# Chemical118/TREW

Measured on AMD Instinct MI355X. Metric: Gbases/s scanned (short 5 32, 150 bp reads), higher is better.
Workload: dtype u32

## Files before the change

### include/trew_hip.h

```cpp
#ifndef TREW_HIP_H
#define TREW_HIP_H

#include <stddef.h>
#include <stdint.h>

#ifdef __cplusplus
extern "C" {
#endif

#define TREW_HIP_ABI_VERSION 4

enum {
    TREW_MODE_SHORT = 0,
    TREW_MODE_PAIR = 1,
    TREW_MODE_LONG = 2,
    TREW_MODE_SEGMENT = 3
};

enum {
    TREW_TABLE_FORWARD_HIGH = 0,
    TREW_TABLE_FORWARD_LOW = 1,
    TREW_TABLE_BACKWARD_HIGH = 2,
    TREW_TABLE_BACKWARD_LOW = 3,
    TREW_TABLE_BOTH_HIGH = 4,
    TREW_TABLE_BOTH_LOW = 5,
    TREW_NUM_TABLES = 6
};

enum {
    TREW_FLAG_NO_FILTER = 1,
    TREW_FLAG_DEBUG_NO_EMIT = 2,
    TREW_FLAG_DEBUG_NO_KLOOP = 4,
    TREW_FLAG_DEBUG_POISON_LDS = 32,
    TREW_FLAG_DEBUG_WIDE_NO_WAIT = 128,
    TREW_FLAG_NO_TIMING = 64,
    TREW_FLAG_COMPAT_G1 = 512,
    TREW_FLAG_DEBUG_NO_JOINT = 2048,
    TREW_FLAG_DEBUG_NO_UNI_DRAIN = 4096,
    TREW_FLAG_DEBUG_NO_GROUP = 1024,
    TREW_FLAG_DEBUG_ANNOT_GENERAL = 8192,
    TREW_FLAG_DEBUG_SMALL_BOUNDS = 16384,
    TREW_FLAG_TRACK_PRESSURE = 256
};

typedef struct {
    int32_t min_mer;
    int32_t max_mer;
    double low_baseline;
    double high_baseline;
    int32_t slice_length;
    int32_t mode;
    int32_t device;
    int32_t n_slots;
    uint64_t max_batch_words;
    uint64_t max_batch_reads;
    uint32_t table_log2_slots;
    uint32_t flags;
    uint64_t max_batch_ascii_bytes;
} trew_hip_params;

typedef struct {
    const uint32_t *words;
    uint64_t n_words;
    const uint32_t *offsets;
    const uint32_t *lengths;
    uint32_t uniform_length;
    uint32_t uniform_stride;
    uint64_t n_reads;
    int32_t on_device;
    int32_t max_length;
} trew_hip_batch;

typedef struct {
    const char *bases;
    uint64_t n_bytes;
    const uint32_t *byte_offsets;
    const uint32_t *lengths;
    const uint32_t *word_offsets;
    uint32_t uniform_length;
    uint32_t reserved;
    uint64_t n_reads;
} trew_hip_ascii_batch;

typedef struct {
    int32_t k;
    int32_t table;
    uint64_t word_lo;
    uint64_t word_hi;
    uint64_t count;
} trew_hip_row;

typedef struct trew_hip_ctx trew_hip_ctx;

int trew_hip_init(const trew_hip_params *params, trew_hip_ctx **out);
void trew_hip_destroy(trew_hip_ctx *ctx);
const char *trew_hip_last_error(const trew_hip_ctx *ctx);

int trew_hip_submit(trew_hip_ctx *ctx, const trew_hip_batch *batch, int slot);
int trew_hip_submit_ascii(trew_hip_ctx *ctx, const trew_hip_ascii_batch *batch, int slot);
int trew_hip_pack_ascii(trew_hip_ctx *ctx, const trew_hip_ascii_batch *batch, uint32_t *words, uint64_t words_cap, uint64_t *n_words);
int trew_hip_wait(trew_hip_ctx *ctx, int slot);

int trew_hip_collect(trew_hip_ctx *ctx, int table, trew_hip_row *rows, uint64_t cap, uint64_t *n_rows);
int trew_hip_reset_tables(trew_hip_ctx *ctx);
int trew_hip_add_rows(trew_hip_ctx *ctx, const trew_hip_row *rows, uint64_t n_rows);

int trew_hip_collect_device(trew_hip_ctx *ctx, trew_hip_row *d_rows, uint64_t cap, uint64_t *n_rows);
int trew_hip_add_rows_device(trew_hip_ctx *ctx, const trew_hip_row *d_rows, uint64_t n_rows);
int trew_hip_merge(trew_hip_ctx *dst, trew_hip_ctx *src);
int trew_hip_add_gathered_device(trew_hip_ctx *ctx, const trew_hip_row *d_buf, uint32_t n_slices, uint32_t own_slice,
                                 uint64_t slice_rows, void *producer_stream, uint64_t *max_rows);
int trew_hip_collect_slice_device(trew_hip_ctx *ctx, trew_hip_row *d_slice, uint64_t slice_rows, void *consumer_stream, uint64_t *n_rows);

int trew_hip_table_pressure(trew_hip_ctx *ctx, uint64_t *used_slots, uint64_t *total_slots, uint64_t *spilled_rows,
                            uint64_t *spill_capacity);

#define TREW_DEBUG_COUNTERS 10
int trew_hip_debug_counters(trew_hip_ctx *ctx, uint64_t *out, int n);

int trew_hip_debug_worklist(trew_hip_ctx *ctx, int slot, uint32_t *units, uint64_t cap, uint64_t *n);

int trew_hip_segment_results(trew_hip_ctx *ctx, int slot, int32_t *k_high, int32_t *k_low,
                             uint64_t *seq_high, uint64_t *seq_low, uint64_t *seq_high_hi, uint64_t *seq_low_hi,
                             uint64_t n_reads);
int trew_hip_filter_masks(trew_hip_ctx *ctx, const trew_hip_batch *batch, uint64_t *cand, int slots_per_read);

int trew_hip_last_timing(trew_hip_ctx *ctx, int slot, float *ms_filter, float *ms_exact, uint64_t *n_flagged);

typedef struct {
    int32_t k;
    int32_t reserved;
    uint64_t word;
} trew_hip_motif;
typedef struct {
    uint32_t windows_fwd, windows_rev, tract_start_fwd, tract_len_fwd, tract_start_rev, tract_len_rev;
} trew_hip_annot;
#define TREW_ANNOT_MAX_MOTIFS 8

int trew_motif_parse(const char *text, trew_hip_motif *out);
int trew_hip_annotate(trew_hip_ctx *ctx, const trew_hip_batch *batch, int slot, const trew_hip_motif *motifs, int n_motifs);
int trew_hip_annotate_results(trew_hip_ctx *ctx, int slot, trew_hip_annot *out, uint64_t cap, uint64_t *n, float *ms_kernel);
int trew_annotate_host(const uint32_t *words, const uint32_t *offsets, const uint32_t *lengths, uint64_t n_reads,
                       const trew_hip_motif *motifs, int n_motifs, trew_hip_annot *out);

typedef struct {
    uint32_t covered_fwd, head_len_fwd, head_cov_fwd, tail_len_fwd, tail_cov_fwd;
    uint32_t covered_rev, head_len_rev, head_cov_rev, tail_len_rev, tail_cov_rev;
} trew_hip_tract;
int trew_hip_tracts(trew_hip_ctx *ctx, const trew_hip_batch *batch, int slot, const trew_hip_motif *motifs, int n_motifs, int penalty);
int trew_hip_tracts_results(trew_hip_ctx *ctx, int slot, trew_hip_tract *out, uint64_t cap, uint64_t *n, float *ms_kernel);
int trew_tracts_host(const uint32_t *words, const uint32_t *offsets, const uint32_t *lengths, uint64_t n_reads,
                     const trew_hip_motif *motifs, int n_motifs, int penalty, trew_hip_tract *out);

typedef struct {
    uint32_t max_gap, min_len;
} trew_hip_interval_rule;
typedef struct {
    uint32_t read, motif, strand, start, end, covered;
} trew_hip_interval;
int trew_hip_intervals(trew_hip_ctx *ctx, const trew_hip_batch *batch, int slot, const trew_hip_motif *motifs, const trew_hip_interval_rule *rules,
                       int n_motifs, uint64_t max_intervals);
int trew_hip_intervals_results(trew_hip_ctx *ctx, int slot, trew_hip_interval *out, uint64_t cap, uint64_t *n, uint32_t *counts, float *ms_kernel);
int trew_intervals_host(const uint32_t *words, const uint32_t *offsets, const uint32_t *lengths, uint64_t n_reads, const trew_hip_motif *motifs,
                        const trew_hip_interval_rule *rules, int n_motifs, trew_hip_interval *out, uint64_t cap, uint64_t *n, uint32_t *counts);

#define TREW_VARIANT_BINS 128
#define TREW_VARIANT_NONE 0xffffffffu
typedef struct {
    uint32_t units_fwd, variants_fwd, distinct_fwd, top_fwd, top_count_fwd;
    uint32_t units_rev, variants_rev, distinct_rev, top_rev, top_count_rev;
} trew_hip_variant;
int trew_hip_variants(trew_hip_ctx *ctx, const trew_hip_batch *batch, int slot, const trew_hip_motif *motifs, int n_motifs);
int trew_hip_variants_results(trew_hip_ctx *ctx, int slot, trew_hip_variant *out, uint64_t cap, uint64_t *n, uint64_t *hist, uint64_t *reads_with,
                              float *ms_kernel);
int trew_variants_host(const uint32_t *words, const uint32_t *offsets, const uint32_t *lengths, uint64_t n_reads, const trew_hip_motif *motifs,
                       int n_motifs, trew_hip_variant *out, uint64_t *hist, uint64_t *reads_with);

typedef struct {
    uint32_t period, scored_period, score, start, end, matches, support, reserved;
    uint64_t unit;
} trew_hip_period;
int trew_hip_periods(trew_hip_ctx *ctx, const trew_hip_batch *batch, int slot, int min_period, int max_period, int penalty, uint32_t min_score);
int trew_hip_periods_results(trew_hip_ctx *ctx, int slot, trew_hip_period *out, uint64_t cap, uint64_t *n, float *ms_kernel);
int trew_periods_host(const uint32_t *words, const uint32_t *offsets, const uint32_t *lengths, uint64_t n_reads, int min_period, int max_period,
                      int penalty, uint32_t min_score, trew_hip_period *out);

typedef struct {
    uint32_t read, motif, strand, start, count, bin;
} trew_hip_chain_item;
int trew_hip_chain(trew_hip_ctx *ctx, const trew_hip_batch *batch, int slot, const trew_hip_motif *motifs, int n_motifs, uint64_t max_events);
int trew_hip_chain_results(trew_hip_ctx *ctx, int slot, trew_hip_chain_item *out, uint64_t cap, uint64_t *n_items, uint64_t *n_events,
                           uint32_t *counts, float *ms_kernel);
int trew_chain_host(const uint32_t *words, const uint32_t *offsets, const uint32_t *lengths, uint64_t n_reads, const trew_hip_motif *motifs,
                    int n_motifs, trew_hip_chain_item *out, uint64_t cap, uint64_t *n_items, uint32_t *counts);

typedef struct {
    uint32_t read, depth, period, scored_period, score, start, end, matches, support, reserved;
    uint64_t unit;
} trew_hip_repeat;
int trew_hip_repeats(trew_hip_ctx *ctx, const trew_hip_batch *batch, int slot, int min_period, int max_period, int penalty, uint32_t min_score,
                     uint64_t max_records);
int trew_hip_repeats_results(trew_hip_ctx *ctx, int slot, trew_hip_repeat *out, uint64_t cap, uint64_t *n, uint32_t *counts, float *ms_kernel);
int trew_repeats_host(const uint32_t *words, const uint32_t *offsets, const uint32_t *lengths, uint64_t n_reads, int min_period, int max_period,
// ... 99 lines not shown
```

### trew_amd/__init__.py

```python
from . import capi
from .capi import (
    FLAG_NO_FILTER,
    FLAG_DEBUG_ANNOT_GENERAL,
    FLAG_DEBUG_POISON_LDS,
    FLAG_NO_TIMING,
    FLAG_TRACK_PRESSURE,
    FLAG_COMPAT_G1,
    FLAG_DEBUG_NO_GROUP,
    FLAG_DEBUG_NO_JOINT,
    FLAG_DEBUG_NO_UNI_DRAIN,
    FLAG_DEBUG_SMALL_BOUNDS,
    FLAG_DEBUG_WIDE_NO_WAIT,
    MODE_LONG,
    MODE_PAIR,
    MODE_SEGMENT,
    MODE_SHORT,
    TABLE_NAMES,
    TrewHip,
    TrewHipError,
    align,
    annotate,
    chain,
    decompose,
    intervals,
    k_mer_check,
    pack_reads,
    periods,
    refine,
    repeats,
    satellites,
    tandems,
    trace,
    tracts,
    variants,
)
```

### trew_amd/capi.py

```python
from __future__ import annotations

import ctypes as C
import os

import numpy as np

_HERE = os.path.dirname(os.path.abspath(__file__))
LIB_PATH = os.environ.get("TREW_HIP_LIB") or os.path.join(_HERE, "lib", "libtrew_hip.so")

MODE_SHORT, MODE_PAIR, MODE_LONG, MODE_SEGMENT = 0, 1, 2, 3
FLAG_NO_FILTER = 1
FLAG_DEBUG_POISON_LDS = 32
FLAG_NO_TIMING = 64
FLAG_COMPAT_G1 = 512
FLAG_TRACK_PRESSURE = 256
FLAG_DEBUG_NO_JOINT = 2048
FLAG_DEBUG_NO_UNI_DRAIN = 4096
FLAG_DEBUG_NO_GROUP = 1024
FLAG_DEBUG_ANNOT_GENERAL = 8192
FLAG_DEBUG_SMALL_BOUNDS = 16384
FLAG_DEBUG_WIDE_NO_WAIT = 128
TABLE_NAMES = ("forward_high", "forward_low", "backward_high", "backward_low", "both_high", "both_low")

EXPORTED_SYMBOLS = (
    "trew_hip_init", "trew_hip_destroy", "trew_hip_last_error", "trew_hip_submit", "trew_hip_wait",
    "trew_hip_collect", "trew_hip_reset_tables", "trew_hip_add_rows", "trew_hip_segment_results",
    "trew_hip_filter_masks", "trew_hip_last_timing", "trew_pack_words", "trew_pack_reads",
    "trew_synth_short_ascii", "trew_synth_short_device", "trew_synth_pair_ascii", "trew_synth_pair_device",
    "trew_hip_malloc", "trew_hip_free", "trew_hip_memcpy_h2d", "trew_hip_memcpy_d2h", "trew_hip_abi_version",
    "trew_pack_pairs", "trew_hip_host_alloc", "trew_hip_host_free", "trew_hip_device_count",
    "trew_synth_long_lengths", "trew_synth_long_ascii", "trew_synth_long_device",
    "trew_hip_collect_device", "trew_hip_add_rows_device", "trew_hip_merge", "trew_hip_table_pressure",
    "trew_hip_add_gathered_device", "trew_hip_collect_slice_device", "trew_hip_debug_counters", "trew_hip_debug_worklist", "trew_hip_submit_ascii", "trew_hip_pack_ascii",
    "trew_motif_parse", "trew_hip_annotate", "trew_hip_annotate_results", "trew_annotate_host",
    "trew_hip_tracts", "trew_hip_tracts_results", "trew_tracts_host",
    "trew_hip_intervals", "trew_hip_intervals_results", "trew_intervals_host",
    "trew_hip_variants", "trew_hip_variants_results", "trew_variants_host",
    "trew_hip_periods", "trew_hip_periods_results", "trew_periods_host",
    "trew_hip_chain", "trew_hip_chain_results", "trew_chain_host",
    "trew_hip_repeats", "trew_hip_repeats_results", "trew_repeats_host",
    "trew_hip_satellites", "trew_hip_satellites_results", "trew_satellites_host",
    "trew_hip_align", "trew_hip_align_results", "trew_align_host",
    "trew_hip_refine", "trew_hip_refine_results", "trew_refine_host",
    "trew_hip_tandems", "trew_hip_tandems_results", "trew_tandems_host",
    "trew_hip_trace", "trew_hip_trace_results", "trew_trace_host",
    "trew_hip_decompose", "trew_hip_decompose_results", "trew_decompose_host",
)
DEBUG_COUNTERS = ("strict_rerun", "windows_fallback", "wide_spin_timeout", "inserted", "inserted_wide", "group_punt", "group_routed", "group_target",
                  "half_drain", "unit_drain")


class Params(C.Structure):
    _fields_ = [
        ("min_mer", C.c_int32), ("max_mer", C.c_int32),
        ("low_baseline", C.c_double), ("high_baseline", C.c_double),
        ("slice_length", C.c_int32), ("mode", C.c_int32), ("device", C.c_int32), ("n_slots", C.c_int32),
        ("max_batch_words", C.c_uint64), ("max_batch_reads", C.c_uint64),
        ("table_log2_slots", C.c_uint32), ("flags", C.c_uint32),
        ("max_batch_ascii_bytes", C.c_uint64),
    ]


class Batch(C.Structure):
    _fields_ = [
        ("words", C.c_void_p), ("n_words", C.c_uint64),
        ("offsets", C.c_void_p), ("lengths", C.c_void_p),
        ("uniform_length", C.c_uint32), ("uniform_stride", C.c_uint32),
        ("n_reads", C.c_uint64), ("on_device", C.c_int32), ("max_length", C.c_int32),
    ]


class AsciiBatch(C.Structure):
    _fields_ = [
        ("bases", C.c_void_p), ("n_bytes", C.c_uint64),
        ("byte_offsets", C.c_void_p), ("lengths", C.c_void_p), ("word_offsets", C.c_void_p),
        ("uniform_length", C.c_uint32), ("reserved", C.c_uint32), ("n_reads", C.c_uint64),
    ]


class Row(C.Structure):
    _fields_ = [("k", C.c_int32), ("table", C.c_int32), ("word_lo", C.c_uint64), ("word_hi", C.c_uint64),
                ("count", C.c_uint64)]


class Motif(C.Structure):
    _fields_ = [("k", C.c_int32), ("reserved", C.c_int32), ("word", C.c_uint64)]


class Annot(C.Structure):
    _fields_ = [("windows_fwd", C.c_uint32), ("windows_rev", C.c_uint32), ("tract_start_fwd", C.c_uint32),
                ("tract_len_fwd", C.c_uint32), ("tract_start_rev", C.c_uint32), ("tract_len_rev", C.c_uint32)]


ANNOT_DTYPE = np.dtype([(name, "<u4") for name, _ in Annot._fields_])
assert ANNOT_DTYPE.itemsize == C.sizeof(Annot)
MAX_MOTIFS = 8


class Tract(C.Structure):
    _fields_ = [(name + sfx, C.c_uint32) for sfx in ("_fwd", "_rev")
                for name in ("covered", "head_len", "head_cov", "tail_len", "tail_cov")]


TRACT_DTYPE = np.dtype([(name, "<u4") for name, _ in Tract._fields_])
assert TRACT_DTYPE.itemsize == C.sizeof(Tract) == 40


class IntervalRule(C.Structure):
    _fields_ = [("max_gap", C.c_uint32), ("min_len", C.c_uint32)]


class Interval(C.Structure):
    _fields_ = [(name, C.c_uint32) for name in ("read", "motif", "strand", "start", "end", "covered")]


INTERVAL_DTYPE = np.dtype([(name, "<u4") for name, _ in Interval._fields_])
assert INTERVAL_DTYPE.itemsize == C.sizeof(Interval) == 24 and C.sizeof(IntervalRule) == 8


class Variant(C.Structure):
    _fields_ = [(name + s, C.c_uint32) for s in ("_fwd", "_rev") for name in ("units", "variants", "distinct", "top", "top_count")]


VARIANT_DTYPE = np.dtype([(name, "<u4") for name, _ in Variant._fields_])
assert VARIANT_DTYPE.itemsize == C.sizeof(Variant) == 40
VARIANT_BINS = 128
VARIANT_NONE = 0xFFFFFFFF


class Period(C.Structure):
    _fields_ = [(name, C.c_uint32) for name in ("period", "scored_period", "score", "start", "end", "matches", "support", "reserved")] + [("unit", C.c_uint64)]

# ... 34 lines not shown
class Alignment(C.Structure):
    _fields_ = [(name + sfx, C.c_uint32) for sfx in ("_fwd", "_rev") for name in ("score", "start", "end", "consumed", "matches")]


ALIGN_DTYPE = np.dtype([(name, "<u4") for name, _ in Alignment._fields_])
assert ALIGN_DTYPE.itemsize == C.sizeof(Alignment) == 40


class TraceItem(C.Structure):
    _fields_ = [(name, C.c_uint32) for name in ("read", "motif", "strand", "start", "bases", "count", "phase", "consumed", "mismatches",
                                                "insertions", "deletions", "reserved")]


TRACE_DTYPE = np.dtype([(name, "<u4") for name, _ in TraceItem._fields_])
assert TRACE_DTYPE.itemsize == C.sizeof(TraceItem) == 48


class Refined(C.Structure):
    _fields_ = [(name, C.c_uint32) for name in ("period", "seed_period", "scored_period", "changed", "score", "start", "end", "consumed", "matches",
                                                "seed_score", "support", "reserved")] + [("unit", C.c_uint64), ("seed_unit", C.c_uint64)]


REFINE_DTYPE = np.dtype([(name, "<u8" if name in ("unit", "seed_unit") else "<u4") for name, _ in Refined._fields_])
assert REFINE_DTYPE.itemsize == C.sizeof(Refined) == 64


class Tandem(C.Structure):
    _fields_ = [("read", C.c_uint32), ("depth", C.c_uint32)] + list(Refined._fields_)


TANDEM_DTYPE = np.dtype([(name, "<u8" if name in ("unit", "seed_unit") else "<u4") for name, _ in Tandem._fields_])
assert TANDEM_DTYPE.itemsize == C.sizeof(Tandem) == 72

ROW_DTYPE = np.dtype([("k", "<i4"), ("table", "<i4"), ("word_lo", "<u8"), ("word_hi", "<u8"), ("count", "<u8")])
assert ROW_DTYPE.itemsize == C.sizeof(Row)

_lib = None


def rows_to_tables(rows):
    out = {name: {} for name in TABLE_NAMES}
    if len(rows) == 0:
        return out
    for t, k, lo, hi, c in zip(rows["table"].tolist(), rows["k"].tolist(), rows["word_lo"].tolist(),
                               rows["word_hi"].tolist(), rows["count"].tolist()):
        out[TABLE_NAMES[t]][(k, (hi << 64) | lo)] = c
    return out


def tables_to_rows(tables):
    items = [(k, t, w & 0xFFFFFFFFFFFFFFFF, w >> 64, c)
             for t, name in enumerate(TABLE_NAMES) for (k, w), c in tables.get(name, {}).items()]
    return np.array(items, dtype=ROW_DTYPE) if items else np.zeros(0, dtype=ROW_DTYPE)


def load():
    global _lib
    if _lib is not None:
        return _lib
    if not os.path.exists(LIB_PATH):
        raise OSError("libtrew_hip.so is not built: run `python -c 'import __graft_entry__ as g; g.build()'`")
    lib = C.CDLL(LIB_PATH)
    vp, u64, i32 = C.c_void_p, C.c_uint64, C.c_int
    lib.trew_hip_abi_version.restype = i32
    lib.trew_hip_init.argtypes = [C.POINTER(Params), C.POINTER(vp)]
    lib.trew_hip_destroy.argtypes = [vp]
    lib.trew_hip_destroy.restype = None
    lib.trew_hip_last_error.argtypes = [vp]
    lib.trew_hip_last_error.restype = C.c_char_p
    lib.trew_hip_submit.argtypes = [vp, C.POINTER(Batch), i32]
    lib.trew_hip_wait.argtypes = [vp, i32]
    lib.trew_hip_submit_ascii.argtypes = [vp, C.POINTER(AsciiBatch), i32]
    lib.trew_hip_pack_ascii.argtypes = [vp, C.POINTER(AsciiBatch), vp, u64, C.POINTER(u64)]
    lib.trew_hip_collect.argtypes = [vp, i32, C.POINTER(Row), u64, C.POINTER(u64)]
    lib.trew_hip_reset_tables.argtypes = [vp]
    lib.trew_hip_add_rows.argtypes = [vp, C.POINTER(Row), u64]
    lib.trew_hip_collect_device.argtypes = [vp, vp, u64, C.POINTER(u64)]
    lib.trew_hip_add_rows_device.argtypes = [vp, vp, u64]
    lib.trew_hip_merge.argtypes = [vp, vp]
    lib.trew_hip_add_gathered_device.argtypes = [vp, vp, C.c_uint32, C.c_uint32, u64, vp, C.POINTER(u64)]
    lib.trew_hip_collect_slice_device.argtypes = [vp, vp, u64, vp, C.POINTER(u64)]
    lib.trew_hip_debug_counters.argtypes = [vp, C.POINTER(u64), i32]
    lib.trew_hip_debug_worklist.argtypes = [vp, i32, vp, u64, C.POINTER(u64)]
    lib.trew_hip_table_pressure.argtypes = [vp, C.POINTER(u64), C.POINTER(u64), C.POINTER(u64), C.POINTER(u64)]
    lib.trew_hip_segment_results.argtypes = [vp, i32, vp, vp, vp, vp, vp, vp, u64]
    lib.trew_hip_filter_masks.argtypes = [vp, C.POINTER(Batch), vp, i32]
    lib.trew_hip_last_timing.argtypes = [vp, i32, C.POINTER(C.c_float), C.POINTER(C.c_float), C.POINTER(u64)]
    lib.trew_motif_parse.argtypes = [C.c_char_p, C.POINTER(Motif)]
    lib.trew_hip_annotate.argtypes = [vp, C.POINTER(Batch), i32, C.POINTER(Motif), i32]
    lib.trew_hip_annotate_results.argtypes = [vp, i32, vp, u64, C.POINTER(u64), C.POINTER(C.c_float)]
    lib.trew_annotate_host.argtypes = [vp, vp, vp, u64, C.POINTER(Motif), i32, vp]
    lib.trew_hip_tracts.argtypes = [vp, C.POINTER(Batch), i32, C.POINTER(Motif), i32, i32]
    lib.trew_hip_tracts_results.argtypes = [vp, i32, vp, u64, C.POINTER(u64), C.POINTER(C.c_float)]
    lib.trew_tracts_host.argtypes = [vp, vp, vp, u64, C.POINTER(Motif), i32, i32, vp]
    lib.trew_hip_intervals.argtypes = [vp, C.POINTER(Batch), i32, C.POINTER(Motif), C.POINTER(IntervalRule), i32, u64]
    lib.trew_hip_intervals_results.argtypes = [vp, i32, vp, u64, C.POINTER(u64), vp, C.POINTER(C.c_float)]
    lib.trew_intervals_host.argtypes = [vp, vp, vp, u64, C.POINTER(Motif), C.POINTER(IntervalRule), i32, vp, u64, C.POINTER(u64), vp]
    lib.trew_hip_variants.argtypes = [vp, C.POINTER(Batch), i32, C.POINTER(Motif), i32]
    lib.trew_hip_variants_results.argtypes = [vp, i32, vp, u64, C.POINTER(u64), vp, vp, C.POINTER(C.c_float)]
    lib.trew_variants_host.argtypes = [vp, vp, vp, u64, C.POINTER(Motif), i32, vp, vp, vp]
    lib.trew_hip_periods.argtypes = [vp, C.POINTER(Batch), i32, i32, i32, i32, C.c_uint32]
    lib.trew_hip_periods_results.argtypes = [vp, i32, vp, u64, C.POINTER(u64), C.POINTER(C.c_float)]
    lib.trew_periods_host.argtypes = [vp, vp, vp, u64, i32, i32, i32, C.c_uint32, vp]
    lib.trew_hip_chain.argtypes = [vp, C.POINTER(Batch), i32, C.POINTER(Motif), i32, u64]
    lib.trew_hip_chain_results.argtypes = [vp, i32, vp, u64, C.POINTER(u64), C.POINTER(u64), vp, C.POINTER(C.c_float)]
    lib.trew_chain_host.argtypes = [vp, vp, vp, u64, C.POINTER(Motif), i32, vp, u64, C.POINTER(u64), vp]
    lib.trew_hip_repeats.argtypes = [vp, C.POINTER(Batch), i32, i32, i32, i32, C.c_uint32, u64]
    lib.trew_hip_repeats_results.argtypes = [vp, i32, vp, u64, C.POINTER(u64), vp, C.POINTER(C.c_float)]
    lib.trew_repeats_host.argtypes = [vp, vp, vp, u64, i32, i32, i32, C.c_uint32, vp, u64, C.POINTER(u64), vp]
    lib.trew_hip_satellites.argtypes = lib.trew_hip_repeats.argtypes
    lib.trew_hip_satellites_results.argtypes = lib.trew_hip_repeats_results.argtypes
    lib.trew_satellites_host.argtypes = lib.trew_repeats_host.argtypes
    lib.trew_hip_align.argtypes = lib.trew_hip_tracts.argtypes
    lib.trew_hip_align_results.argtypes = lib.trew_hip_tracts_results.argtypes
    lib.trew_align_host.argtypes = lib.trew_tracts_host.argtypes
    lib.trew_hip_trace.argtypes = [vp, C.POINTER(Batch), i32, C.POINTER(Motif), i32, i32, C.c_uint32, u64, u64]
    lib.trew_hip_trace_results.argtypes = [vp, i32, vp, u64, C.POINTER(u64), C.POINTER(u64), vp, vp, C.POINTER(C.c_float)]
    lib.trew_trace_host.argtypes = [vp, vp, vp, u64, C.POINTER(Motif), i32, i32, C.c_uint32, vp, u64, C.POINTER(u64), vp, vp]
    lib.trew_hip_decompose.argtypes = [vp, C.POINTER(Batch), i32, i32, i32, i32, C.c_uint32, u64, u64]
    lib.trew_hip_decompose_results.argtypes = lib.trew_hip_trace_results.argtypes
    lib.trew_decompose_host.argtypes = [vp, vp, vp, u64, i32, i32, i32, C.c_uint32, vp, u64, C.POINTER(u64), vp, vp]
    lib.trew_hip_refine.argtypes = lib.trew_hip_periods.argtypes
    lib.trew_hip_refine_results.argtypes = lib.trew_hip_periods_results.argtypes
    lib.trew_refine_host.argtypes = lib.trew_periods_host.argtypes
    lib.trew_hip_tandems.argtypes = lib.trew_hip_repeats.argtypes
    lib.trew_hip_tandems_results.argtypes = lib.trew_hip_repeats_results.argtypes
    lib.trew_tandems_host.argtypes = lib.trew_repeats_host.argtypes
    lib.trew_pack_words.argtypes = [u64]
    lib.trew_pack_words.restype = u64
    lib.trew_pack_reads.argtypes = [C.c_char_p, vp, vp, u64, vp, u64, vp, vp]
    lib.trew_pack_reads.restype = u64
    lib.trew_synth_short_ascii.argtypes = [u64, u64, u64, C.c_uint32, vp]
    lib.trew_synth_short_device.argtypes = [vp, u64, u64, u64, C.c_uint32, vp]
    lib.trew_synth_pair_ascii.argtypes = [u64, u64, u64, C.c_uint32, vp, vp]
    lib.trew_synth_pair_device.argtypes = [vp, u64, u64, u64, C.c_uint32, vp]
    lib.trew_synth_long_lengths.argtypes = [u64, u64, u64, vp]
    lib.trew_synth_long_ascii.argtypes = [u64, u64, u64, vp, vp]
    lib.trew_synth_long_device.argtypes = [vp, u64, u64, u64, vp, vp]
    lib.trew_hip_malloc.argtypes = [vp, u64, C.POINTER(vp)]
    lib.trew_hip_free.argtypes = [vp, vp]
    lib.trew_hip_memcpy_h2d.argtypes = [vp, vp, vp, u64]
    lib.trew_hip_memcpy_d2h.argtypes = [vp, vp, vp, u64]
    _lib = lib
    return lib


class TrewHipError(RuntimeError):
    pass


def pack_reads(reads):
    lib = load()
    reads = [r.encode() if isinstance(r, str) else bytes(r) for r in reads]
    n = len(reads)
    st = np.zeros(n, dtype=np.int64)
    nd = np.zeros(n, dtype=np.int64)
    pos = 0
    for i, r in enumerate(reads):
        st[i] = pos
        nd[i] = pos + len(r) - 1
        pos += len(r) + 1
    buf = b"\n".join(reads) + b"\n"
    cap = int(sum(lib.trew_pack_words(len(r)) for r in reads)) + 8
    words = np.zeros(cap, dtype=np.uint32)
    offsets = np.zeros(max(n, 1), dtype=np.uint32)
    lengths = np.zeros(max(n, 1), dtype=np.uint32)
# ... 593 lines not shown
        counts = np.zeros(n_reads, dtype=np.uint32)
        records = np.zeros(n_reads, dtype=REFINE_DTYPE)
        self._chk(self.lib.trew_hip_decompose_results(self.ctx, slot, None, 0, C.byref(n_items), C.byref(n_rows), counts.ctypes.data, records.ctypes.data,
                                                      C.byref(ms) if want_ms else None), "trew_hip_decompose_results")
        items, rows = int(n_items.value), int(n_rows.value)
        out = np.zeros(items if items <= max_items and rows <= max_rows else 0, dtype=TRACE_DTYPE)
        if len(out):
            self._chk(self.lib.trew_hip_decompose_results(self.ctx, slot, out.ctypes.data, len(out), C.byref(n_items), C.byref(n_rows), None, None, None),
                      "trew_hip_decompose_results")
        return (out, counts, records, items, rows, ms.value) if want_ms else (out, counts, records, items, rows)

    def repeats(self, batch, min_period=1, max_period=32, penalty=3, min_score=24, max_records=None, slot=0):
        self._queue_tracts("repeats", batch, min_period, max_period, penalty, min_score, max_records, slot)

    def repeats_results(self, slot=0, want_ms=False):
        return self._fetch_log("repeats", slot, REPEAT_DTYPE, want_ms)

    def tandems(self, batch, min_period=1, max_period=32, penalty=3, min_score=24, max_records=None, slot=0):
        self._queue_tracts("tandems", batch, min_period, max_period, penalty, min_score, max_records, slot)

    def tandems_results(self, slot=0, want_ms=False):
        return self._fetch_log("tandems", slot, TANDEM_DTYPE, want_ms)

    def satellites(self, batch, min_period=1, max_period=SATELLITE_MAX_PERIOD, penalty=3, min_score=24, max_records=None, slot=0):
        self._queue_tracts("satellites", batch, min_period, max_period, penalty, min_score, max_records, slot)

    def satellites_results(self, slot=0, want_ms=False):
        return self._fetch_log("satellites", slot, SATELLITE_DTYPE, want_ms)

    def submit_reads(self, reads, slot=0):
        b = self.host_batch(*pack_reads(reads))
        self.submit(b, slot)
        return b

    def collect_rows(self, table=-1):
        n = C.c_uint64(0)
        cap = getattr(self, "_collect_cap", 1 << 16)
        while True:
            rows = np.zeros(cap, dtype=ROW_DTYPE)
            self._chk(self.lib.trew_hip_collect(self.ctx, table, C.cast(rows.ctypes.data, C.POINTER(Row)), cap,
                                                C.byref(n)), "trew_hip_collect")
            if n.value <= cap:
                return rows[: n.value]
            cap = self._collect_cap = int(n.value) + 1024

    def collect(self):
        return rows_to_tables(self.collect_rows(-1))

    def reset_tables(self):
        self._chk(self.lib.trew_hip_reset_tables(self.ctx), "trew_hip_reset_tables")

    def add_rows(self, tables):
        rows = tables if isinstance(tables, np.ndarray) else tables_to_rows(tables)
        rows = np.ascontiguousarray(rows, dtype=ROW_DTYPE)
        if len(rows):
            self._chk(self.lib.trew_hip_add_rows(self.ctx, C.cast(rows.ctypes.data, C.POINTER(Row)), len(rows)),
                      "trew_hip_add_rows")

    def collect_device(self, d_rows, cap):
        n = C.c_uint64(0)
        self._chk(self.lib.trew_hip_collect_device(self.ctx, d_rows, cap, C.byref(n)), "trew_hip_collect_device")
        return int(n.value)

    def collect_slice_device(self, d_slice, slice_rows, consumer_stream=None, want_count=False):
        n = C.c_uint64(0)
        self._chk(self.lib.trew_hip_collect_slice_device(self.ctx, d_slice, slice_rows, consumer_stream, C.byref(n) if want_count else None),
                  "trew_hip_collect_slice_device")
        return int(n.value) if want_count else None

    def add_rows_device(self, d_rows, n_rows):
        self._chk(self.lib.trew_hip_add_rows_device(self.ctx, d_rows, n_rows), "trew_hip_add_rows_device")

    def add_gathered_device(self, d_buf, n_slices, own_slice, slice_rows, producer_stream=None):
        mx = C.c_uint64(0)
        self._chk(self.lib.trew_hip_add_gathered_device(self.ctx, d_buf, n_slices, own_slice, slice_rows, producer_stream, C.byref(mx)),
                  "trew_hip_add_gathered_device")
        return int(mx.value)

    def debug_counters(self):
        out = (C.c_uint64 * len(DEBUG_COUNTERS))()
        self._chk(self.lib.trew_hip_debug_counters(self.ctx, out, len(DEBUG_COUNTERS)), "trew_hip_debug_counters")
        return dict(zip(DEBUG_COUNTERS, (int(x) for x in out)))

    def debug_worklist(self, slot=0):
        n = C.c_uint64(0)
        self._chk(self.lib.trew_hip_debug_worklist(self.ctx, slot, None, 0, C.byref(n)), "trew_hip_debug_worklist")
        out = np.zeros(int(n.value), dtype=np.uint32)
        if len(out):
            self._chk(self.lib.trew_hip_debug_worklist(self.ctx, slot, out.ctypes.data, len(out), C.byref(n)), "trew_hip_debug_worklist")
        return out

    def merge_from(self, other):
        self._chk(self.lib.trew_hip_merge(self.ctx, other.ctx), "trew_hip_merge")

    def table_pressure(self):
        v = [C.c_uint64(0) for _ in range(4)]
        self._chk(self.lib.trew_hip_table_pressure(self.ctx, *[C.byref(x) for x in v]), "trew_hip_table_pressure")
        return tuple(int(x.value) for x in v)

    def segment_results(self, n_reads, slot=0):
        kh = np.zeros(n_reads, dtype=np.int32)
        kl = np.zeros(n_reads, dtype=np.int32)
        sh = np.zeros(n_reads, dtype=np.uint64)
        sl = np.zeros(n_reads, dtype=np.uint64)
        shh = np.zeros(n_reads, dtype=np.uint64)
        slh = np.zeros(n_reads, dtype=np.uint64)
        self._chk(self.lib.trew_hip_segment_results(self.ctx, slot, kh.ctypes.data, kl.ctypes.data, sh.ctypes.data,
                                                    sl.ctypes.data, shh.ctypes.data, slh.ctypes.data, n_reads),
                  "trew_hip_segment_results")
        seq_h = [(int(a) << 64) | int(b) for a, b in zip(shh, sh)]
        seq_l = [(int(a) << 64) | int(b) for a, b in zip(slh, sl)]
        return kh, kl, seq_h, seq_l

    def filter_masks(self, batch, slots_per_read):
        units = batch.n_reads // 2 if self.mode == MODE_PAIR else batch.n_reads
        cand = np.zeros(max(1, units * slots_per_read), dtype=np.uint64)
        self._chk(self.lib.trew_hip_filter_masks(self.ctx, C.byref(batch), cand.ctypes.data, slots_per_read),
                  "trew_hip_filter_masks")
        return cand[: units * slots_per_read].reshape(units, slots_per_read)

    def last_timing(self, slot=0, want_flagged=True):
        a, b, n = C.c_float(), C.c_float(), C.c_uint64()
        self._chk(self.lib.trew_hip_last_timing(self.ctx, slot, C.byref(a), C.byref(b), C.byref(n) if want_flagged else None),
                  "trew_hip_last_timing")
        return a.value, b.value, n.value

    def malloc(self, nbytes):
        p = C.c_void_p()
        self._chk(self.lib.trew_hip_malloc(self.ctx, nbytes, C.byref(p)), "trew_hip_malloc")
        return p.value

    def free(self, ptr):
        self._chk(self.lib.trew_hip_free(self.ctx, ptr), "trew_hip_free")

    def d2h(self, ptr, nbytes):
        out = np.zeros(nbytes, dtype=np.uint8)
        self._chk(self.lib.trew_hip_memcpy_d2h(self.ctx, out.ctypes.data, ptr, nbytes), "trew_hip_memcpy_d2h")
        return out

    def synth_short_device(self, seed, first_read, n_reads, read_len, d_words):
        self._chk(self.lib.trew_synth_short_device(self.ctx, seed, first_read, n_reads, read_len, d_words),
                  "trew_synth_short_device")

    def synth_long_device(self, seed, first_read, n_reads):
        lens = synth_long_lengths(seed, first_read, n_reads)
        nw = 3 * ((lens.astype(np.int64) + 31) // 32)
        offs = np.zeros(n_reads, dtype=np.int64)
        offs[1:] = np.cumsum(nw[:-1])
        total = int(offs[-1] + nw[-1]) if n_reads else 0
        if total >= 2 ** 32:
            raise TrewHipError("long batch exceeds 2^32 words")
        offs32 = offs.astype(np.uint32)
        d_words = self.malloc(total * 4 + 64)
        d_offs = self.malloc(n_reads * 4)
        d_lens = self.malloc(n_reads * 4)
        self._chk(self.lib.trew_hip_memcpy_h2d(self.ctx, d_offs, offs32.ctypes.data, n_reads * 4), "h2d")
        self._chk(self.lib.trew_hip_memcpy_h2d(self.ctx, d_lens, lens.ctypes.data, n_reads * 4), "h2d")
        self._chk(self.lib.trew_synth_long_device(self.ctx, seed, first_read, n_reads, d_offs, d_words), "trew_synth_long_device")
        b = Batch(d_words, total, d_offs, d_lens, 0, 0, n_reads, 1, int(lens.max()) if n_reads else 0)
        return b, (d_words, d_offs, d_lens), int(lens.astype(np.int64).sum())

    def synth_pair_device(self, seed, first_pair, n_pairs, read_len, d_words):
        self._chk(self.lib.trew_synth_pair_device(self.ctx, seed, first_pair, n_pairs, read_len, d_words),
                  "trew_synth_pair_device")


def k_mer_check(seq, min_mer=5, max_mer=32, low=0.5, high=0.8, flags=0, device=0):
    if isinstance(seq, str):
        seq = seq.encode()
    with TrewHip(mode=MODE_SEGMENT, min_mer=min_mer, max_mer=max_mer, low=low, high=high, device=device, n_slots=1,
                 max_batch_words=1 << 12, max_batch_reads=16, table_log2_slots=14, flags=flags) as t:
        t.submit_reads([seq])
        t.wait()
# ... 114 lines not shown
```

### trew_amd/csrc/kernels/bound.inc

```


template <bool POS = false>
__device__ __forceinline__ u32 low_mask(int bits) {
    return bits >= 32 ? 0xffffffffu : ((!POS && bits <= 0) ? 0u : ((1u << bits) - 1u));
}

__device__ __forceinline__ u32 word_parity(u32 x) {
    x ^= x << 1;
    x ^= x << 2;
    x ^= x << 4;
    x ^= x << 8;
    x ^= x << 16;
    return x;
}

template <int NW>
__device__ __forceinline__ void prefix_parity(const u32 (&f)[NW], u32 (&P)[NW]) {
    u32 carry = 0, prev_top = 0;
#pragma unroll
    for (int j = 0; j < NW; j++) {
        const u32 x = word_parity(f[j]) ^ carry;
        P[j] = (x << 1) | prev_top;
        prev_top = x >> 31;
        carry = 0u - prev_top;
// ... 53 lines not shown
}

template <int NW>
__device__ __forceinline__ void windows_without_n(const u32 (&v1)[NW], bool has_n, int L, int k, int bmax, u32 (&V)[NW]) {
    if (!has_n) {
        const int wbits = L - k + 1;
#pragma unroll
        for (int j = 0; j < NW; j++) V[j] = low_mask(wbits - 32 * j);
    } else {
        u32 A[NW];
#pragma unroll
        for (int j = 0; j < NW; j++) {
            V[j] = 0xffffffffu;
            A[j] = v1[j];
        }
        u32 off = 0;
#pragma unroll
        for (int b = 1; b <= 64; b <<= 1) {
            if (b > 1) {
                u32 T2[NW];
#pragma unroll
                for (int j = 0; j < NW; j++) T2[j] = A[j] & shr_var_word<NW>(A, j, (u32) (b / 2));
#pragma unroll
                for (int j = 0; j < NW; j++) A[j] = T2[j];
            }
            if (b <= bmax) {
                const bool take = ((u32) k & (u32) b) != 0;
#pragma unroll
                for (int j = 0; j < NW; j++) {
                    const u32 sh = shr_var_word<NW>(A, j, off);
                    V[j] &= take ? sh : 0xffffffffu;
                }
                off += take ? (u32) b : 0u;
            }
        }
    }
}

template <bool MASKED, bool COUNTED>
struct Buckets8 {
    u32 c000 = 0, c001 = 0, c010 = 0, c011 = 0, c100 = 0, c101 = 0, c110 = 0, c111 = 0, count = 0;
    __device__ __forceinline__ void add(u32 F1, u32 F2, u32 F3, u32 v) {
        u32 a11, a10, a01, a00;
        if (MASKED) {
            a11 = F1 & F2, a10 = F1 & ~F2, a01 = ~F1 & F2, a00 = v & ~(F1 | F2);
        } else {
            const u32 a1 = v & F1, a0 = v ^ a1;
            a11 = a1 & F2, a10 = a1 ^ a11, a01 = a0 & F2, a00 = a0 ^ a01;
        }
        const u32 b111 = a11 & F3, b101 = a10 & F3, b011 = a01 & F3, b001 = a00 & F3;
        if (!COUNTED) count += __popc(v);
        c111 += __popc(b111);
        c110 += __popc(a11 ^ b111);
        c101 += __popc(b101);
        c100 += __popc(a10 ^ b101);
        c011 += __popc(b011);
        c010 += __popc(a01 ^ b011);
        c001 += __popc(b001);
        if (!COUNTED) c000 += __popc(a00 ^ b001);
    }
    __device__ __forceinline__ u32 largest(u32 known = 0) {
        if (COUNTED) c000 = known - c001 - c010 - c011 - c100 - c101 - c110 - c111;
        return max(max(max(c000, c001), max(c010, c011)), max(max(c100, c101), max(c110, c111)));
    }
};
template <int N>
__device__ __forceinline__ u32 max_bucket8(const u32 (&F1)[N], const u32 (&F2)[N], const u32 (&F3)[N], const u32 (&V)[N], u32 count) {
    Buckets8<true, true> b;
#pragma unroll
    for (int j = 0; j < N; j++) b.add(F1[j], F2[j], F3[j], V[j]);
    return b.largest(count);
}

template <int NW>
__device__ __forceinline__ u32 class_links(const u32 (&V)[NW], const u32 (&E)[NW]) {
    u32 links = 0;
#pragma unroll
    for (int j = 0; j < NW; j++) {
        const u32 vn = j + 1 < NW ? V[j + 1 < NW ? j + 1 : 0] : 0u;
        links += __popc(V[j] & E[j] & alignbit(vn, V[j], 1u));
    }
    return links;
}
```

### trew_amd/csrc/kernels/bounds_pass.inc

```

constexpr u32 kBoundsTileStride = kBoundWords + 1;

__device__ __forceinline__ u32 pack_bound_word(u32 m8, u32 count, u32 links, u32 has_n, int k, int gmax, const DevParams &P) {
    const u32 runs = count - links < 127u ? count - links : 127u;
    const double dm = (double) m8, dc = (double) count;
    const double tl = P.low * dc, th = P.high * dc;
    u32 pass_lo = dm > tl ? 1u : 0u, pass_hi = dm > th ? 1u : 0u;
    const bool amb = fabs(dm - tl) <= 1e-9 || fabs(dm - th) <= 1e-9;
    if (__any(amb)) {
        const double ub = count ? dm / dc : 0.0;
        pass_lo = ub >= P.low ? 1u : 0u;
        pass_hi = ub >= P.high ? 1u : 0u;
    }
    const bool inr = k <= gmax && count != 0u;
    return inr ? (m8 | (count << 10) | (runs << 20) | (pass_lo << 27) | (pass_hi << 28) | (has_n << 29)) : (has_n << 29);
}

template <int NW>
__global__ __launch_bounds__(64) void bounds_kernel(DevParams P, DevBatch B, const u32 *__restrict__ wl, const u32 *__restrict__ wl_count, u32 wl_cap,
                                                    u32 *__restrict__ bnd, u32 bnd_cap) {
    static_assert(NW == 3, "the k loop is written for three words: halves of at most 95 bases");
    __shared__ u32 tile[64 * kBoundsTileStride];
    const u32 lane = lane_id();
    u32 n = wl_count[0];
    n = n < wl_cap ? n : wl_cap;
    n = n < bnd_cap ? n : bnd_cap;
    const u64 total = 2ull * n;
    const int klo = P.min_mer, khi = P.max_mer < P.min_mer + (int) kBoundWords - 1 ? P.max_mer : P.min_mer + (int) kBoundWords - 1;
    for (u64 base = (u64) blockIdx.x * 64u; base < total; base += (u64) gridDim.x * 64u) {
        const u64 idx = base + lane;
        const bool active = idx < total;
        const u32 half = (u32) idx & 1u;
        ReadRef rd;
        rd.w = B.words;
        rd.len = rd.nw = 0;
        if (active) rd = get_read(B, wl[idx >> 1]);
        const Segment sg = get_segment(TREW_MODE_SHORT, (int) half, rd.len, 0, P.min_mer, P.max_mer, P.slice_len);
        const bool can = active && sg.valid && sg.len <= 32u * NW - 1u;
        if (!can) rd.nw = 0;
        const int L = can ? (int) sg.len : 0;
        u32 lo[3], hi[3], nm[3], V[3], P1[3], P2[3], P3[3];
        load_planes<3>(rd, sg.start, lo, hi, nm);
        segment_setup<3, false, true, true>(lo, hi, nm, L, V, P1, P2, P3);
        const u32 has_n = segment_has_n<3>(nm, L) != 0u ? 1u : 0u;
        for (int t = 1; t < klo; t++) drain_v_step3(V);
        const int Lmax = (int) wave_max_u32((u32) L);
        u32 *const row = tile + lane * kBoundsTileStride;
        int k = klo;
        for (const int b = khi < Lmax - 64 ? khi : Lmax - 64; k <= b; k++) {
            const u32 bs = (u32) k;
            u32 F1[3], F2[3], F3[3], E[3];
#pragma unroll
            for (int j = 0; j < 3; j++) {
                const int jn = j < 2 ? j + 1 : 0;
                F1[j] = xor_and(P1[j], alignbit(j < 2 ? P1[jn] : 0u, P1[j], bs), V[j]);
                F2[j] = xor_and(P2[j], alignbit(j < 2 ? P2[jn] : 0u, P2[j], bs), V[j]);
                F3[j] = P3[j] ^ alignbit(j < 2 ? P3[jn] : 0u, P3[j], bs);
                E[j] = ~((lo[j] ^ alignbit(j < 2 ? lo[jn] : 0u, lo[j], bs)) | (hi[j] ^ alignbit(j < 2 ? hi[jn] : 0u, hi[j], bs)));
            }
            const u32 count = bcnt_acc(V[2], bcnt_acc(V[1], __popc(V[0])));
            const u32 m8 = max_bucket8<3>(F1, F2, F3, V, count);
            row[k - klo] = pack_bound_word(m8, count, class_links<3>(V, E), has_n, k, P.max_mer, P);
            drain_v_step3(V);
        }
        if (k <= khi) {
            const int o = L > 63 ? L - 63 : 0;
            const u64 Q1 = container64(P1, o), Q2 = container64(P2, o), Q3 = container64(P3, o), Ql = container64(lo, o), Qh = container64(hi, o);
            u64 Vq = ((u64) V[1] << 32) | V[0];
            for (; k <= khi; k++) {
                const u32 sh = (u32) (k - o);
                const u64 S1 = Q1 >> sh, S2 = Q2 >> sh, S3 = Q3 >> sh, Sl = Ql >> sh, Sh = Qh >> sh;
                const u32 Vw[2] = {(u32) Vq, (u32) (Vq >> 32)};
                const u32 F1[2] = {xor_and(P1[0], (u32) S1, Vw[0]), xor_and(P1[1], (u32) (S1 >> 32), Vw[1])};
                const u32 F2[2] = {xor_and(P2[0], (u32) S2, Vw[0]), xor_and(P2[1], (u32) (S2 >> 32), Vw[1])};
                const u32 F3[2] = {P3[0] ^ (u32) S3, P3[1] ^ (u32) (S3 >> 32)};
                const u32 E[2] = {~((lo[0] ^ (u32) Sl) | (hi[0] ^ (u32) Sh)), ~((lo[1] ^ (u32) (Sl >> 32)) | (hi[1] ^ (u32) (Sh >> 32)))};
                const u32 count = bcnt_acc(Vw[1], __popc(Vw[0]));
                const u32 m8 = max_bucket8<2>(F1, F2, F3, Vw, count);
                row[k - klo] = pack_bound_word(m8, count, class_links<2>(Vw, E), has_n, k, P.max_mer, P);
                Vq &= Vq >> 1;
            }
        }
        for (int ki = khi >= klo ? khi - klo + 1 : 0; ki < (int) kBoundWords; ki++) row[ki] = has_n << 29;
        lds_sync();
        const u64 left = total - base;
        const u32 words = (left < 64u ? (u32) left : 64u) * kBoundWords;
        u32 *const dst = bnd + base * kBoundWords;
#pragma unroll 4
        for (u32 r = 0; r < kBoundWords; r++) {
            const u32 w = r * 64u + lane;
            if (w < words) dst[w] = tile[(w >> 5) * kBoundsTileStride + (w & 31u)];
        }
        lds_sync();
    }
}
```

### trew_amd/csrc/kernels/decide_group.inc

```

#define TREW_REGION_LIST(X) \
    X(chunk) X(stage) X(group_setup) X(bounds) X(group) X(dg_loop) X(dg_pick) X(dg_eval) X(er_gaps) X(er_runs) X(er_canon) X(er_merge) X(er_max) \
    X(dg_decision) X(dg_end) X(routing) X(records) X(target) X(target_rows) X(target_eval) X(target_emit) X(fallback)
#define TREW_REGION_ENUM(n) kRegion_##n,
enum { TREW_REGION_LIST(TREW_REGION_ENUM) kRegionCount };
#ifdef TREW_REGION_COUNTS
__device__ unsigned long long g_region[64];
#define TREW_MARK(n)                                                                   \
    do {                                                                               \
        asm volatile("; MARK " #n);                                                    \
        if (lane_id() == 0) atomicAdd(&g_region[kRegion_##n], 1ull);                   \
    } while (0)
#else
#define TREW_MARK(n) asm volatile("; MARK " #n)
#endif
__device__ __forceinline__ void lds_sync() {
    __builtin_amdgcn_fence(__ATOMIC_RELEASE, "wavefront");
    __builtin_amdgcn_wave_barrier();
    __builtin_amdgcn_fence(__ATOMIC_ACQUIRE, "wavefront");
}
#define TREW_DPP(v, ctrl) ((u32) __builtin_amdgcn_update_dpp(0, (int) (v), (ctrl), 0xf, 0xf, false))
__device__ __forceinline__ u32 swap16(u32 v) { return (u32) __builtin_amdgcn_ds_swizzle((int) v, 0x401F); }
template <int G = 16>
__device__ __forceinline__ u32 row_or(u32 v) {
// ... 402 lines not shown
        o.kept_canon = acc ? canon : o.kept_canon;
        o.kept_cnt = acc ? rc.cnt : o.kept_cnt;
        {
            const u32 hit0 = acc & (sk0 >> 8) & 3u, hit1 = acc & (sk1 >> 8) & 3u;
            const u32 bad0 = (__umul24(maxc, skb0 >> 16) < __umul24(skb0 & 0xffffu, count) ? 1u : 0u) | ((skm0 >> kidx) & 1u);
            const u32 bad1 = (__umul24(maxc, skb1 >> 16) < __umul24(skb1 & 0xffffu, count) ? 1u : 0u) | ((skm1 >> kidx) & 1u);
            viol |= (hit0 ? bad0 : 0u) | (hit1 ? bad1 : 0u);
            sk0 |= hit0 << 10;
            sk1 |= hit1 << 10;
        }
        if (__any(acc)) {
            todo &= eligible();
            if (!__any(todo != 0u && punt == 0u)) break;
        }
    }
    TREW_MARK(dg_end);
    viol |= ((sk0 >> 8) & 3u & ~((sk0 >> 10) & 3u)) | ((sk1 >> 8) & 3u & ~((sk1 >> 10) & 3u));
    o.punt = (punt | viol) != 0u;
    PH_ADD(PH_DECIDE, t_ph);
    return o;
}

__device__ __forceinline__ void stage_two(ExactSmem sm, const ReadRef &rdA, const ReadRef &rdB, bool haveB) {
    const u32 lane = lane_id();
    lds_sync();
    const u32 r = lane >> 5, segwords = exact_rangewords(sm.cap);
    ReadRef rr;
    rr.w = r ? rdB.w : rdA.w;
    rr.len = r ? rdB.len : rdA.len;
    rr.nw = r ? rdB.nw : rdA.nw;
    const u32 L = rr.len;
    u64 *seq = sm_seq(sm) + r * segwords;
    u32 *nmk = sm_nmask(sm) + r * segwords;
    const u32 nwords = (L + 31u) >> 5;
    if (r == 0u || haveB) {
        for (u32 l = lane & 31u; l < segwords; l += 32u) {
            u64 sq = 0;
            u32 nmv = 0xffffffffu;
            if (l < nwords) {
                u32 lo1[1], hi1[1], nm1[1];
                load_planes_lds<1>(rr, 32u * l, lo1, hi1, nm1);
                nmv = nm1[0] | ~low_mask<true>((int) L - 32 * (int) l);
                const u32 lq = lo1[0] & ~nmv, hq = hi1[0] & ~nmv;
                sq = spread32(__brev(lq)) | (spread32(__brev(hq)) << 1);
            }
            seq[l] = sq;
            nmk[l] = nmv;
        }
    }
    lds_sync();
}

template <typename WT>
__device__ __forceinline__ WT strand_canon(WT w, int k) {
    const WT rc = min_rotation<WT>(revcomp(w, k), k);
    return rc < w ? rc : w;
}

template <typename WT>
__device__ __forceinline__ WT strand_flip(WT w, int k) {
    return min_rotation<WT>(revcomp(w, k), k);
}

constexpr u32 kBoundWords = 32;
constexpr u32 kBoundItemWords = 2 * kBoundWords;
struct NoStoredBounds {
    static constexpr bool kAny = false;
};
struct StoredBounds {
    static constexpr bool kAny = true;
    u32 posA, posB;
};
struct ExactKernArgs {
    DevParams P;
    DevBatch B;
    DevTableG1 TG;
    const u32 *wl;
    u32 *wl_count, *wl_count_next;
    u32 wl_cap;
    SegResults R;
    u32 cap, rawwords;
    const u32 *bnd;
    u32 bnd_cap;
};
template <int NW, typename WT, typename SB>
__device__ void run_short_group(ExactSmem sm, const DevParams &P, TableRef T, const ReadRef rdA, const ReadRef rdB, bool haveB, const SB sb) {
    const u32 lane = lane_id();
#if defined(TREW_AB_SKIP) && TREW_AB_SKIP >= 5
    return;
#endif
    u32 st0 = 0, st1 = 0;
    bool stored = false;
    if constexpr (SB::kAny) {
        typedef const __attribute__((address_space(4))) u64 *c64;
        typedef const __attribute__((address_space(4))) u32 *c32;
        const u64 ka = (u64) __builtin_amdgcn_kernarg_segment_ptr();
        const u32 bcap = *(c32) (ka + offsetof(ExactKernArgs, bnd_cap));
        const u32 posA = rfl(sb.posA), posB = rfl(sb.posB);
        stored = posA < bcap && posB < bcap;
        if (stored && (lane < 32u || haveB)) {
            const u32 *const base = (const u32 *) *(c64) (ka + offsetof(ExactKernArgs, bnd));
            const u32 *src = base + ((u64) (lane < 32u ? posA : posB) * 2u + ((lane >> 4) & 1u)) * kBoundWords + (lane & 15u);
            st0 = src[0];
            st1 = src[16];
        }
    }
    TREW_MARK(stage);
    PH_T0(t_stage);
    stage_two(sm, rdA, rdB, haveB);
    PH_ADD(PH_STAGE, t_stage);
#if defined(TREW_AB_SKIP) && TREW_AB_SKIP >= 4
    return;
#endif
    TREW_MARK(group_setup);
    const u32 g = lane >> 4, j = lane & 15u;
    const bool second = g >= 2u;
    const u32 is_right = g & 1u;
    ReadRef rd;
    rd.w = second ? rdB.w : rdA.w;
    rd.len = second ? rdB.len : rdA.len;
    rd.nw = second ? rdB.nw : rdA.nw;
    const Segment sg = get_segment(TREW_MODE_SHORT, (int) is_right, rd.len, 0, P.min_mer, P.max_mer, P.slice_len);
    const bool rowvalid = sg.valid && (!second || haveB);
    TREW_MARK(bounds);
    PH_T0(t_bounds);
    RowSeg<NW> rs;
    u32 bnd0, bnd1;
    if (stored) {
        u32 nm[NW];
        ReadRef r = rd;
        if (!rowvalid) r.nw = 0;
        load_planes_lds<NW>(r, sg.start, rs.lo, rs.hi, nm);
        u32 anyn = 0;
#pragma unroll
        for (int w = 0; w < NW; w++) {
            rs.v1[w] = ~nm[w] & low_mask((int) sg.len - 32 * w);
            rs.P1[w] = rs.P2[w] = rs.P3[w] = 0;
            anyn |= ~rs.v1[w] & low_mask((int) sg.len - 32 * w);
        }
        rs.has_n = anyn != 0u ? 1u : 0u;
        bnd0 = rowvalid ? st0 : 0u;
        bnd1 = rowvalid ? st1 : 0u;
    } else {
        lds_sync();
        row_prepare<NW>(sm, rd, sg, rowvalid);
        lds_sync();
        row_load<NW>(sm, (int) sg.len, rs);
        if (P.min_mer + 15 < 32)
            bnd0 = rowvalid ? bound_at_k<NW, true>(rs, (int) sg.len, P.min_mer + (int) j, P.max_mer, P) : 0u;
        else
            bnd0 = rowvalid ? bound_at_k<NW, false>(rs, (int) sg.len, P.min_mer + (int) j, P.max_mer, P) : 0u;
        bnd1 = rowvalid ? bound_at_k<NW>(rs, (int) sg.len, P.min_mer + 16 + (int) j, P.max_mer, P) : 0u;
    }
#if defined(TREW_AB_SKIP) && TREW_AB_SKIP >= 3
    asm volatile("" ::"v"(bnd0), "v"(bnd1));
    return;
#endif
    PH_ADD(PH_BOUNDS, t_bounds);
    TREW_MARK(group);
    const GroupOut<WT> o = decide_group<NW, WT, false>(sm, P, rs, bnd0, bnd1, second ? 1u : 0u, sg, rowvalid);
#if defined(TREW_AB_SKIP) && TREW_AB_SKIP >= 2
    asm volatile("" ::"v"(o.kk), "v"(o.saved), "v"(o.kept_cnt), "v"((u32) o.kept_canon), "v"((u32) (o.kept_canon >> 32)), "v"((u32) o.punt));
    return;
#endif
    TREW_MARK(routing);
    PH_T0(t_route);
    const u32 mine = rowvalid ? (o.kk | (o.punt ? 1u << 16 : 0u)) : 0u;
    const u32 other = lane_gather(mine, lane ^ 16u);
    const u32 kkL = is_right ? other : mine, kkR = is_right ? mine : other;
    const u32 lkh = kkL & 255u, lkl = (kkL >> 8) & 255u, rkh = kkR & 255u, rkl = (kkR >> 8) & 255u;
    const u32 left_found = (lkh | lkl) != 0u ? 1u : 0u;
    const u32 tgt_h = left_found & (lkh == rkh ? 1u : 0u) & (lkh != 0u ? 1u : 0u);
    const u32 tgt_l = left_found & (lkl == rkl ? 1u : 0u) & (lkl != 0u ? 1u : 0u);
    const u32 myk = o.saved & 255u, items = (o.saved >> 8) & 255u;
    u32 need_old = ((kkL | kkR) >> 16) & 1u;
    u32 rec_mask = 0;
    {
        const u32 kh = is_right ? rkh : lkh, kl = is_right ? rkl : lkl;
        const u32 rec_h = (kh != 0u ? 1u : 0u) & (is_right ? ((left_found ^ 1u) | (lkh == 0u ? 1u : 0u)) : (tgt_h ^ 1u));
        const u32 rec_l = (kl != 0u ? 1u : 0u) & (is_right ? ((left_found ^ 1u) | (lkl == 0u ? 1u : 0u)) : (tgt_l ^ 1u));
// ... 134 lines not shown
```

### trew_amd/csrc/kernels/exact_kernel.inc

```

#ifndef TREW_EXACT_SHORT_WAVES
#define TREW_EXACT_SHORT_WAVES 5
#endif
#ifndef TREW_EXACT_PAIR_WAVES
#define TREW_EXACT_PAIR_WAVES 4
#endif
#ifndef TREW_EXACT_LONG_WAVES
#define TREW_EXACT_LONG_WAVES 4
#endif
template <int NW, int MODE>
constexpr int exact_waves(bool narrow) {
    return NW >= 10 ? 4
                    : (narrow && NW > 0 && MODE == TREW_MODE_SHORT
                           ? TREW_EXACT_SHORT_WAVES
                           : (narrow && NW > 0 && MODE == TREW_MODE_PAIR ? TREW_EXACT_PAIR_WAVES : (narrow && NW == 5 && MODE == TREW_MODE_LONG ? TREW_EXACT_LONG_WAVES : 6)));
}
template <int NW, int MODE, typename WT>
__global__ __launch_bounds__(64, (exact_waves<NW, MODE>(sizeof(WT) == 8))) void exact_kernel(DevParams P, DevBatch B, DevTableG1 TG, const u32 *wl,
                                                   u32 *wl_count, u32 *wl_count_next, u32 wl_cap, SegResults R, u32 cap, u32 rawwords,
                                                   const u32 *bnd, u32 bnd_cap) {
    typedef ExactKernArgs KernArgs;
    static_assert(alignof(DevParams) == 8 && alignof(DevBatch) == 8 && alignof(DevTableG1) == 8, "kernarg layout: 8-byte aligned argument structs");
    static_assert(sizeof(DevParams) % 8 == 0 && sizeof(DevBatch) % 8 == 0, "kernarg layout: no padding between the argument structs");
    static_assert(offsetof(KernArgs, TG) == sizeof(DevParams) + sizeof(DevBatch), "kernarg layout: TG follows P and B");
    static_assert(offsetof(DevTableG1, t) == 0, "TableRef points at DevTableG1::t");
    const TableRef T = (TableRef) ((const char *) __builtin_amdgcn_kernarg_segment_ptr() + offsetof(KernArgs, TG));
#ifdef TREW_AB_EXACT_PRIO
    __builtin_amdgcn_s_setprio(TREW_AB_EXACT_PRIO);
#endif
    if (blockIdx.x == 0 && wl_count_next) {
        for (u32 i = lane_id(); i < (1u + 8u) * 32u; i += 64u) wl_count_next[i] = 0u;
    }
    ExactSmem sm;
    sm.lds = lds_offset_in_kernel();
    sm.cap = cap;
    sm.rawwords = rawwords;
    sm.s0 = 0;
    sm.rs = sm.rnw = 0;
    sm.rw = nullptr;
    u32 n = wl_count[0];
    n = n < wl_cap ? n : wl_cap;
#ifdef TREW_PHASE_PROFILE
    if (lane_id() < 32) ph_lds()[lane_id()] = 0;
    __syncthreads();
#endif
    PH_T0(t_total);
    if (P.flags & TREW_FLAG_DEBUG_POISON_LDS) {
        if (blockIdx.x == 0 && lane_id() == 0) {
            const u32 *through = (const u32 *) T, *byval = (const u32 *) &TG;
            bool same = true;
            for (u32 i = 0; i < sizeof(DevTableG1) / 4; i++) same = same && through[i] == byval[i];
            if (!same) atomicAdd(&TG.t.overflow[kDiagKernarg], 1u);
        }
        const u32 nb = exact_lds_bytes(cap, rawwords, sizeof(WT));
        for (u32 i = lane_id() * 4u; i < nb; i += 256u) *(u32 *) (lds0() + i) = 0xA5C3F00Du ^ (i * 2654435761u);
        __syncthreads();
    }
    cache_clear(sm);
    const bool use_group = P.max_mer - P.min_mer < 32 && !(P.flags & TREW_FLAG_DEBUG_NO_GROUP);
    if (use_group) group_fill_multiples(sm, P);
    constexpr u32 kChunk = MODE == TREW_MODE_LONG ? 1 : 4, kShards = 8, kHeadStride = 32;
    u32 *heads = wl_count + kHeadStride;
    const u32 my = blockIdx.x & (kShards - 1);
    const u32 lane = lane_id();
    if constexpr (MODE == TREW_MODE_SHORT || MODE == TREW_MODE_SEGMENT || MODE == TREW_MODE_PAIR) {
        constexpr u32 kMetaWords = 32;
        constexpr u32 kPer = MODE == TREW_MODE_PAIR ? 2u : 1u;
        constexpr u32 kUnits = kChunk / kPer;
        u32 *const meta_base = sm_intent(sm);
        u32 *const raw_base = sm_raw(sm);
        u32 sh = my, shards_tried = 0, cpend = 0;
        auto issue_claim = [&]() __attribute__((always_inline)) {
            if (lane == 0) cpend = atomicAdd(&heads[sh * kHeadStride], 1u);
        };
        auto resolve_claim = [&]() __attribute__((always_inline)) -> u64 {
            u32 c = rfl(cpend);
            for (;;) {
                const u64 w0l = ((u64) c * kShards + sh) * kUnits;
                if (w0l < n) return w0l;
                u32 seen = 0;
                do {
                    if (++shards_tried >= kShards) return ~0ull;
                    sh = (sh + 1u) & (kShards - 1u);
                    seen = rfl(__hip_atomic_load(&heads[sh * kHeadStride], __ATOMIC_RELAXED, __HIP_MEMORY_SCOPE_AGENT));
                } while (((u64) seen * kShards + sh) * kUnits >= n);
                u32 c2 = 0;
                if (lane == 0) c2 = atomicAdd(&heads[sh * kHeadStride], 1u);
                c = rfl(c2);
            }
        };
        auto chunk_items = [&](u64 w0l) __attribute__((always_inline)) -> u32 { return (u32) ((w0l + kUnits < n ? w0l + kUnits : n) - w0l); };
        auto fetch_units = [&](u32 bf, u64 w0l, u32 nit) __attribute__((always_inline)) {
            if (lane < nit) __builtin_amdgcn_global_load_lds(wl + w0l + lane, (__attribute__((address_space(3))) u32 *) (meta_base + bf * kMetaWords), 4, 0, 0);
        };
        auto fetch_words = [&](u32 bf, u32 nit) __attribute__((always_inline)) {
            typedef const __attribute__((address_space(4))) u64 *c64;
            typedef const __attribute__((address_space(4))) u32 *c32;
            const u64 ka = (u64) __builtin_amdgcn_kernarg_segment_ptr() + offsetof(KernArgs, B);
            DevBatch Bk;
            Bk.words = (const u32 *) *(c64) (ka + offsetof(DevBatch, words));
            Bk.offsets = (const u32 *) *(c64) (ka + offsetof(DevBatch, offsets));
            Bk.lengths = (const u32 *) *(c64) (ka + offsetof(DevBatch, lengths));
            Bk.uniform_length = *(c32) (ka + offsetof(DevBatch, uniform_length));
            Bk.uniform_stride = *(c32) (ka + offsetof(DevBatch, uniform_stride));
            u32 *meta = meta_base + bf * kMetaWords;
            const bool mine = lane < nit * kPer;
            const u64 read_l = mine ? (u64) meta[lane / kPer] * kPer + lane % kPer : 0ull;
            u64 off_l = 0;
            u32 len_l = 0;
            if (mine) {
                off_l = Bk.offsets ? (u64) Bk.offsets[read_l] : read_l * (u64) Bk.uniform_stride;
                len_l = Bk.lengths ? Bk.lengths[read_l] : Bk.uniform_length;
            }
            if (lane < kChunk) {
                meta[4 + lane] = len_l;
                meta[8 + lane] = (u32) off_l;
                meta[12 + lane] = (u32) (off_l >> 32);
                meta[16 + lane] = 3u * ((len_l + 31u) >> 5) <= sm.rawwords ? 1u : 0u;
            }
#pragma unroll
            for (u32 t = 0; t < kChunk; t++) {
                const u64 off = readlane_word(off_l, (int) t);
                const u32 nwords = 3u * (((u32) __builtin_amdgcn_readlane((int) len_l, (int) t) + 31u) >> 5);
                if (nwords <= sm.rawwords) {
                    u32 *dst = raw_base + (bf * kChunk + t) * sm.rawwords;
                    for (u32 j0 = 0; j0 < nwords; j0 += 64u)
                        if (j0 + lane < nwords) __builtin_amdgcn_global_load_lds(Bk.words + off + j0 + lane, (__attribute__((address_space(3))) u32 *) (dst + j0), 4, 0, 0);
                }
            }
        };
        auto landed = [&]() __attribute__((always_inline)) {
            __builtin_amdgcn_s_waitcnt(0);
            __syncthreads();
        };
        u32 bf = 0;
        PH_T0(t_stage0);
        issue_claim();
        u64 cur = resolve_claim();
        if (cur != ~0ull) {
            fetch_units(0, cur, chunk_items(cur));
            landed();
            fetch_words(0, chunk_items(cur));
            issue_claim();
            landed();
        }
        PH_ADD(PH_STAGE, t_stage0);
        constexpr bool kGroup = MODE == TREW_MODE_SHORT && sizeof(WT) == 8 && (NW == 3 || NW == 5);
        bool grouped = false;
        if constexpr (kGroup) grouped = use_group;
        while (cur != ~0ull) {
            TREW_MARK(chunk);
            const u32 nit = chunk_items(cur);
            u32 *const meta = meta_base + bf * kMetaWords;
            PH_T0(t_p0);
            const u64 nxt = resolve_claim();
            PH_ADD(PH_STAGE, t_p0);
            const u32 nxt_nit = nxt != ~0ull ? chunk_items(nxt) : 0u;
            if (nxt_nit) fetch_units(bf ^ 1u, nxt, nxt_nit);
            const u32 hook = nit < kUnits / 2u ? nit : kUnits / 2u;
            PH_CNT(PH_N_READS, nit);
            auto item = [&](u32 t, ReadRef &rd, u32 &unit, bool &staged) __attribute__((always_inline)) {
                rd.len = rfl(meta[4 + t]);
                rd.nw = (rd.len + 31u) >> 5;
                unit = rfl(meta[t / kPer]);
                const u64 off = ((u64) rfl(meta[12 + t]) << 32) | rfl(meta[8 + t]);
                staged = rfl(meta[16 + t]) != 0u;
                rd.w = staged ? (const u32 *) (raw_base + (bf * kChunk + t) * sm.rawwords) : B.words + off;
            };
            ReadRef held;
            held.w = nullptr;
            held.len = held.nw = 0;
            bool have_held = false;
            u32 held_pos = 0;
            for (u32 t = 0; t <= nit; t++) {
                if (t == hook && nxt_nit) {
                    PH_T0(t_p1);
// ... 130 lines not shown
```

### trew_amd/csrc/trew_capi.cpp

```cpp
#include <hip/hip_runtime.h>

#include <algorithm>
#include <atomic>
#include <cmath>
#include <cstdio>
#include <cstdlib>
#include <cstring>
#include <mutex>
#include <string>
#include <thread>
#include <vector>

#include "trew_common.hpp"
#include "trew_launch.hpp"
#include "trew_measures_host.hpp"
#include "trew_synth.hpp"

using namespace trew;

namespace {

enum Measure { kAnnotate, kTracts, kIntervals, kVariants, kPeriods, kChain, kRepeats, kSatellites, kAlign, kRefine, kTandems, kTrace, kDecompose, kMeasures };
const char *const kMeasureName[kMeasures] = {"annotate", "tracts", "intervals", "variants", "periods", "chain", "repeats", "satellites", "align", "refine", "tandems", "trace", "decompose"};
const bool kMeasureHasMotifs[kMeasures] = {true, true, true, true, false, true, false, false, true, false, false, true, false};
struct DevBuf {
    void *p = nullptr;
    u64 bytes = 0;
};
struct MeasureState {
    DevBuf records;
    DevBuf counts;
    unsigned long long *counter = nullptr;
    unsigned long long *hist = nullptr;
    hipEvent_t ev[2] = {nullptr, nullptr};
    bool valid = false, timed = false;
    u64 n = 0;
    u64 max_log = 0;
    u64 n_counts = 0;
    int n_motifs = 0;
    u32 k[kAnnotMaxMotifs] = {};
    DevBuf rows;
    DevBuf aligned;
    u64 max_rows = 0;
};

struct Slot {
    hipStream_t stream = nullptr;
    u32 *d_buf = nullptr;
    u32 *d_words = nullptr, *d_offsets = nullptr, *d_lengths = nullptr;
    unsigned char *d_ascii = nullptr;
    u32 *d_wl = nullptr;
    u32 *d_wl_count = nullptr;
    u32 *d_bnd = nullptr;
    u32 bnd_cap = 0;
    int2 *d_thr = nullptr;
    int2 *h_thr = nullptr;
    hipEvent_t ev_tail = nullptr, ev_copied = nullptr;
    u32 *h_seen = nullptr;
    u32 thr_length = 0;
    SegResults res = {nullptr, nullptr, nullptr, nullptr};
    static constexpr int kRing = 128;
    hipEvent_t ev[kRing][3] = {};
    u64 n_launches = 0;
    u64 n_submits = 0;
    u64 n_reported = 0;
    u64 n_units = 0;
    AnnotMotifDev *d_motifs = nullptr, *h_motifs = nullptr;
    int motifs_staged = 0;
    MeasureState measure[kMeasures];
};

thread_local std::string g_init_error;
thread_local std::string g_thread_error;
constexpr size_t kWlCountWords = 32 + 8 * 32;
constexpr size_t kWlCountBytes = kWlCountWords * 4;

}

struct trew_hip_ctx {
    trew_hip_params p;
    DevParams dp;
    DevTable table;
    DevTableG1 table_g1;
    DevG1 g1 = {nullptr, nullptr, nullptr, 0};
    trew_hip_row *g1_carry[2] = {nullptr, nullptr};
    u32 g1_carry_cap = 0;
    u64 g1_batches = 0;
    DevWide wide;
    u64 table_slots = 0;
    std::vector<Slot> slots;
    hipStream_t copy_stream = nullptr;
    std::mutex copy_mu;
    hipStream_t fill_stream = nullptr;
    hipEvent_t ev_filled = nullptr;
    int n_cu = 256;
    unsigned long long *d_collect_n = nullptr;
    trew_hip_row *d_collect_rows = nullptr;
    u64 collect_cap = 0;
    trew_hip_row *d_add_rows = nullptr;
    u64 add_cap = 0;
    u32 *d_row_flags = nullptr;
    hipEvent_t ev_producer = nullptr;
    std::mutex table_mu;
    std::atomic<u32> seen[kDiagWords];
    std::atomic<int> last_slot{-1};
    std::mutex seen_mu;
};

static void note_seen(trew_hip_ctx *ctx, const u32 *diag) {
    for (int i : {(int) kDiagOverflow, (int) kDiagInserted, (int) kDiagInsertedWide, (int) kDiagSpillRows}) {
        u32 cur = ctx->seen[i].load(std::memory_order_relaxed);
        while (cur < diag[i] && !ctx->seen[i].compare_exchange_weak(cur, diag[i], std::memory_order_relaxed)) {
        }
    }
}

#define HIPCHK(ctx, expr)                                                                         \
    do {                                                                                          \
        hipError_t e_ = (expr);                                                                   \
        if (e_ != hipSuccess) {                                                                   \
            (void) (ctx);                                                                         \
            g_thread_error = std::string(#expr) + ": " + hipGetErrorString(e_);                   \
            return (int) e_ ? (int) e_ : -1;                                                      \
        }                                                                                         \
    } while (0)

static int fail(trew_hip_ctx *, const std::string &msg) {
    g_thread_error = msg;
    return -1;
}

extern "C" int trew_hip_abi_version(void) { return TREW_HIP_ABI_VERSION; }

extern "C" int trew_hip_device_count(void) {
    int n = 0;
    return hipGetDeviceCount(&n) == hipSuccess ? n : 0;
}

extern "C" int trew_hip_host_alloc(trew_hip_ctx *ctx, uint64_t bytes, void **h_ptr) {
    if (!ctx || !h_ptr) return -1;
    hipError_t e = hipSetDevice(ctx->p.device);
    if (e == hipSuccess) e = hipHostMalloc(h_ptr, bytes, hipHostMallocDefault);
    if (e != hipSuccess) {
        g_thread_error = std::string("hipHostMalloc: ") + hipGetErrorString(e);
        return (int) e;
    }
    return 0;
}

extern "C" int trew_hip_host_free(trew_hip_ctx *ctx, void *h_ptr) {
    if (!ctx) return -1;
    hipError_t e = hipHostFree(h_ptr);
    if (e != hipSuccess) {
        g_thread_error = std::string("hipHostFree: ") + hipGetErrorString(e);
        return (int) e;
    }
    return 0;
}

extern "C" const char *trew_hip_last_error(const trew_hip_ctx *ctx) {
    return ctx ? g_thread_error.c_str() : g_init_error.c_str();
}

static float conservative_lowf(double low) {
    float f = (float) (low * (1.0 - 1e-6));
    f = std::nextafterf(f, 0.0f);
    return f;
}

static int order_behind_fills(trew_hip_ctx *ctx) {
    HIPCHK(ctx, hipEventRecord(ctx->ev_filled, ctx->fill_stream));
    for (auto &s : ctx->slots)
        if (s.stream) HIPCHK(ctx, hipStreamWaitEvent(s.stream, ctx->ev_filled, 0));
    return 0;
}

extern "C" int trew_hip_init(const trew_hip_params *params, trew_hip_ctx **out) {
    if (!params || !out) {
        g_init_error = "trew_hip_init: null argument";
        return -1;
    }
    *out = nullptr;
    const trew_hip_params &p = *params;
    if (p.min_mer > p.max_mer) { g_init_error = "MIN_MER must not be greater than MAX_MER."; return -1; }
    if (p.min_mer < 3) { g_init_error = "MIN_MER must be greater than or equal to 3."; return -1; }
    if (p.max_mer > 64) { g_init_error = "MAX_MER must be less than or equal to 64."; return -1; }
    if (!(0 < p.low_baseline && p.low_baseline <= 1) || !(0 < p.high_baseline && p.high_baseline <= 1)) { g_init_error = "Baseline must be in range 0 to 1."; return -1; }
    if (p.low_baseline > p.high_baseline) { g_init_error = "Low baseline must be smaller than high baseline."; return -1; }
// ... 9 lines not shown
    if (p.n_slots < 1 || p.n_slots > 512) { g_init_error = "n_slots must be in [1,512]"; return -1; }
    if (p.table_log2_slots < 12 || p.table_log2_slots > 30) { g_init_error = "table_log2_slots must be in [12,30]"; return -1; }
    if (p.max_batch_reads == 0 || p.max_batch_reads > 0xfffffff0ull) { g_init_error = "max_batch_reads out of range"; return -1; }

    int ndev = 0;
    hipError_t e = hipGetDeviceCount(&ndev);
    if (e != hipSuccess || ndev <= 0) {
        g_init_error = std::string("no HIP device available: ") + hipGetErrorString(e);
        return -2;
    }
    if (p.device < 0 || p.device >= ndev) { g_init_error = "device ordinal out of range"; return -1; }
    e = hipSetDevice(p.device);
    if (e != hipSuccess) { g_init_error = std::string("hipSetDevice: ") + hipGetErrorString(e); return -2; }

    trew_hip_ctx *ctx = new trew_hip_ctx();
    for (auto &v : ctx->seen) v.store(0, std::memory_order_relaxed);
    memset(&ctx->table, 0, sizeof(ctx->table));
    memset(&ctx->wide, 0, sizeof(ctx->wide));
    ctx->p = p;
    ctx->dp.min_mer = p.min_mer;
    ctx->dp.max_mer = p.max_mer;
    ctx->dp.low = p.low_baseline;
    ctx->dp.high = p.high_baseline;
    ctx->dp.lowf = conservative_lowf(p.low_baseline);
    ctx->dp.slice_len = p.slice_length > 0 ? p.slice_length : 150;
    ctx->dp.mode = p.mode;
    ctx->dp.flags = p.flags;
    hipDeviceProp_t prop;
    if (hipGetDeviceProperties(&prop, p.device) == hipSuccess) ctx->n_cu = prop.multiProcessorCount;

    auto bail = [&](const char *what, hipError_t er) {
        g_init_error = std::string(what) + ": " + hipGetErrorString(er);
        trew_hip_destroy(ctx);
        return -3;
    };
    if ((e = hipStreamCreateWithFlags(&ctx->copy_stream, hipStreamNonBlocking)) != hipSuccess) return bail("hipStreamCreate", e);
    ctx->fill_stream = ctx->copy_stream;
    if ((e = hipEventCreateWithFlags(&ctx->ev_filled, hipEventDisableTiming)) != hipSuccess) return bail("hipEventCreate", e);
    ctx->table_slots = 1ull << p.table_log2_slots;
    ctx->table.log2_part_slots = p.table_log2_slots - kTablePartBits;
    if ((e = hipMalloc((void **) &ctx->table.keys, ctx->table_slots * 8)) != hipSuccess) return bail("hipMalloc(table keys)", e);
    if ((e = hipMalloc((void **) &ctx->table.counts, ctx->table_slots * 8)) != hipSuccess) return bail("hipMalloc(table counts)", e);
    if ((e = hipMalloc((void **) &ctx->table.overflow, kDiagWords * 4)) != hipSuccess) return bail("hipMalloc(overflow)", e);
    if ((e = hipMemsetAsync(ctx->table.keys, 0, ctx->table_slots * 8, ctx->fill_stream)) != hipSuccess) return bail("hipMemsetAsync", e);
    if ((e = hipMemsetAsync(ctx->table.counts, 0, ctx->table_slots * 8, ctx->fill_stream)) != hipSuccess) return bail("hipMemsetAsync", e);
    if ((e = hipMemsetAsync(ctx->table.overflow, 0, kDiagWords * 4, ctx->fill_stream)) != hipSuccess) return bail("hipMemsetAsync", e);
    ctx->wide.wide_log2_slots = std::max<u32>(10u, p.table_log2_slots - 2u);
    {
        const size_t wb = (size_t) 8 << ctx->wide.wide_log2_slots;
        u64 **arr[4] = {&ctx->wide.wtag, &ctx->wide.wlo, &ctx->wide.whi, &ctx->wide.wcount};
        for (auto a : arr) {
            if ((e = hipMalloc((void **) a, wb)) != hipSuccess) return bail("hipMalloc(wide table)", e);
            if ((e = hipMemsetAsync(*a, 0, wb, ctx->fill_stream)) != hipSuccess) return bail("hipMemsetAsync", e);
        }
        ctx->wide.spill_cap = (u32) std::max<u64>(1ull << 16, ctx->table_slots >> 4);
        ctx->wide.spin_limit = (p.flags & TREW_FLAG_DEBUG_WIDE_NO_WAIT) ? 0u : (1u << 20);
        if ((e = hipMalloc((void **) &ctx->wide.spill_rows, (size_t) ctx->wide.spill_cap * sizeof(trew_hip_row))) != hipSuccess) return bail("hipMalloc(spill log)", e);
        ctx->wide.spill_n = ctx->table.overflow + kDiagSpillRows;
        DevWide *dw = nullptr;
        if ((e = hipMalloc((void **) &dw, sizeof(DevWide))) != hipSuccess) return bail("hipMalloc(wide descriptor)", e);
        if ((e = hipMemcpy(dw, &ctx->wide, sizeof(DevWide), hipMemcpyHostToDevice)) != hipSuccess) return bail("hipMemcpy", e);
        ctx->table.wide = dw;
    }
    {
        if (p.flags & TREW_FLAG_COMPAT_G1) {
            ctx->g1.log_cap = (u32) std::min<u64>(std::max<u64>(1ull << 16, 24ull * (p.max_batch_reads / 2)), 1ull << 26);
            ctx->g1_carry_cap = 1u << 16;
            if ((e = hipMalloc((void **) &ctx->g1.log, (size_t) ctx->g1.log_cap * sizeof(trew_hip_row))) != hipSuccess) return bail("hipMalloc(G1 log)", e);
            if ((e = hipMalloc((void **) &ctx->g1.counters, 16)) != hipSuccess) return bail("hipMalloc(G1 counters)", e);
            if ((e = hipMemsetAsync(ctx->g1.counters, 0, 16, ctx->fill_stream)) != hipSuccess) return bail("hipMemsetAsync", e);
            if ((e = hipMalloc((void **) &ctx->g1.pair_flags, (size_t) (p.max_batch_reads / 2 + 64))) != hipSuccess) return bail("hipMalloc(G1 pair flags)", e);
            for (auto &cb : ctx->g1_carry)
                if ((e = hipMalloc((void **) &cb, (size_t) ctx->g1_carry_cap * sizeof(trew_hip_row))) != hipSuccess) return bail("hipMalloc(G1 carry)", e);
        }
        DevTableG1 tbl;
        tbl.t = ctx->table;
        tbl.g = ctx->g1;
        tbl.w = ctx->wide;
        if (p.flags & TREW_FLAG_DEBUG_NO_EMIT) tbl.t.log2_part_slots = 0xffffffffu;
        ctx->table_g1 = tbl;
    }

    if ((e = hipMalloc((void **) &ctx->d_row_flags, kRowFlagWords * 4)) != hipSuccess) return bail("hipMalloc(row flags)", e);
    if ((e = hipEventCreateWithFlags(&ctx->ev_producer, hipEventDisableTiming)) != hipSuccess) return bail("hipEventCreate", e);
    ctx->slots.resize((size_t) p.n_slots);
    for (auto &s : ctx->slots) {
        if ((e = hipStreamCreateWithFlags(&s.stream, hipStreamNonBlocking)) != hipSuccess) return bail("hipStreamCreate", e);
        if ((e = hipEventCreateWithFlags(&s.ev_tail, hipEventDisableTiming)) != hipSuccess) return bail("hipEventCreate", e);
        if ((e = hipEventCreateWithFlags(&s.ev_copied, hipEventDisableTiming)) != hipSuccess) return bail("hipEventCreate", e);
        {
            const size_t words = 2 * (size_t) p.max_batch_reads + (size_t) p.max_batch_words + 8;
            if ((e = hipMalloc((void **) &s.d_buf, words * 4)) != hipSuccess) return bail("hipMalloc(batch buffer)", e);
            if ((e = hipMemsetAsync(s.d_buf, 0, words * 4, ctx->fill_stream)) != hipSuccess) return bail("hipMemsetAsync", e);
            s.d_offsets = s.d_buf;
            s.d_lengths = s.d_buf + p.max_batch_reads;
            s.d_words = s.d_buf + 2 * (size_t) p.max_batch_reads;
        }
        if (p.max_batch_ascii_bytes) {
            if ((e = hipMalloc((void **) &s.d_ascii, p.max_batch_ascii_bytes + 256)) != hipSuccess) return bail("hipMalloc(text buffer)", e);
            if ((e = hipMemsetAsync(s.d_ascii, 0, p.max_batch_ascii_bytes + 256, ctx->fill_stream)) != hipSuccess) return bail("hipMemsetAsync", e);
        }
        if ((e = hipMalloc((void **) &s.d_thr, kThrTableBytes)) != hipSuccess) return bail("hipMalloc(thresholds)", e);
        if ((e = hipHostMalloc((void **) &s.h_thr, kThrTableBytes + kDiagWords * 4, hipHostMallocDefault)) != hipSuccess) return bail("hipHostMalloc(thresholds)", e);
        s.h_seen = (u32 *) ((char *) s.h_thr + kThrTableBytes);
        memset(s.h_seen, 0, kDiagWords * 4);
        if ((e = hipMalloc((void **) &s.d_wl, p.max_batch_reads * sizeof(u32))) != hipSuccess) return bail("hipMalloc(worklist)", e);
        if (bounds_pass_applies(ctx->dp, 1)) {
            const u64 share = std::min<u64>(std::max<u64>(p.max_batch_reads / 32, std::min<u64>(p.max_batch_reads, 1ull << 16)), 1ull << 22);
            s.bnd_cap = (p.flags & TREW_FLAG_DEBUG_SMALL_BOUNDS) ? 64u : (u32) share;
            if ((e = hipMalloc((void **) &s.d_bnd, (size_t) s.bnd_cap * bounds_entry_bytes())) != hipSuccess) return bail("hipMalloc(bounds)", e);
        }
        if ((e = hipMalloc((void **) &s.d_wl_count, 2 * kWlCountBytes)) != hipSuccess) return bail("hipMalloc(wl_count)", e);
        if ((e = hipMemsetAsync(s.d_wl_count, 0, 2 * kWlCountBytes, ctx->fill_stream)) != hipSuccess) return bail("hipMemsetAsync", e);
        if (p.mode == TREW_MODE_SEGMENT) {
            if ((e = hipMalloc((void **) &s.res.k_high, p.max_batch_reads * 4)) != hipSuccess) return bail("hipMalloc", e);
            if ((e = hipMalloc((void **) &s.res.k_low, p.max_batch_reads * 4)) != hipSuccess) return bail("hipMalloc", e);
            if ((e = hipMalloc((void **) &s.res.seq_high, p.max_batch_reads * 8)) != hipSuccess) return bail("hipMalloc", e);
            if ((e = hipMalloc((void **) &s.res.seq_low, p.max_batch_reads * 8)) != hipSuccess) return bail("hipMalloc", e);
            if ((e = hipMalloc((void **) &s.res.seq_high_hi, p.max_batch_reads * 8)) != hipSuccess) return bail("hipMalloc", e);
            if ((e = hipMalloc((void **) &s.res.seq_low_hi, p.max_batch_reads * 8)) != hipSuccess) return bail("hipMalloc", e);
        }
        for (int i = 0; i < Slot::kRing; i++)
            for (int j = 0; j < 3; j++)
                if ((e = hipEventCreate(&s.ev[i][j])) != hipSuccess) return bail("hipEventCreate", e);
    }
    if (int rc = order_behind_fills(ctx)) {
        g_init_error = g_thread_error;
        trew_hip_destroy(ctx);
        return rc;
    }
    *out = ctx;
    return 0;
}

extern "C" void trew_hip_destroy(trew_hip_ctx *ctx) {
    if (!ctx) return;
    (void) hipSetDevice(ctx->p.device);
    for (auto &s : ctx->slots) {
        if (s.stream) (void) hipStreamSynchronize(s.stream);
        if (s.d_buf) (void) hipFree(s.d_buf);
        if (s.d_ascii) (void) hipFree(s.d_ascii);
        if (s.d_thr) (void) hipFree(s.d_thr);
        if (s.h_thr) (void) hipHostFree(s.h_thr);
        if (s.d_wl) (void) hipFree(s.d_wl);
        if (s.d_bnd) (void) hipFree(s.d_bnd);
        if (s.d_wl_count) (void) hipFree(s.d_wl_count);
        if (s.res.k_high) (void) hipFree(s.res.k_high);
        if (s.res.k_low) (void) hipFree(s.res.k_low);
        if (s.res.seq_high) (void) hipFree(s.res.seq_high);
        if (s.res.seq_low) (void) hipFree(s.res.seq_low);
        if (s.res.seq_high_hi) (void) hipFree(s.res.seq_high_hi);
        if (s.res.seq_low_hi) (void) hipFree(s.res.seq_low_hi);
        for (int i = 0; i < Slot::kRing; i++)
            for (int j = 0; j < 3; j++)
                if (s.ev[i][j]) (void) hipEventDestroy(s.ev[i][j]);
        if (s.d_motifs) (void) hipFree(s.d_motifs);
        if (s.h_motifs) (void) hipHostFree(s.h_motifs);
        for (auto &st : s.measure) {
            for (void *p : {st.records.p, st.counts.p, st.rows.p, st.aligned.p, (void *) st.counter, (void *) st.hist})
                if (p) (void) hipFree(p);
            for (auto e : st.ev)
                if (e) (void) hipEventDestroy(e);
        }
        if (s.ev_tail) (void) hipEventDestroy(s.ev_tail);
        if (s.ev_copied) (void) hipEventDestroy(s.ev_copied);
        if (s.stream) (void) hipStreamDestroy(s.stream);
    }
    if (ctx->copy_stream) (void) hipStreamSynchronize(ctx->copy_stream);
    if (ctx->copy_stream) (void) hipStreamDestroy(ctx->copy_stream);
    if (ctx->ev_filled) (void) hipEventDestroy(ctx->ev_filled);
    if (ctx->table.keys) (void) hipFree(ctx->table.keys);
    if (ctx->table.counts) (void) hipFree(ctx->table.counts);
    if (ctx->table.overflow) (void) hipFree(ctx->table.overflow);
    if (ctx->wide.wtag) (void) hipFree(ctx->wide.wtag);
    if (ctx->wide.wlo) (void) hipFree(ctx->wide.wlo);
    if (ctx->wide.whi) (void) hipFree(ctx->wide.whi);
    if (ctx->wide.wcount) (void) hipFree(ctx->wide.wcount);
    if (ctx->wide.spill_rows) (void) hipFree(ctx->wide.spill_rows);
    if (ctx->table.wide) (void) hipFree((void *) ctx->table.wide);
    if (ctx->g1.log) (void) hipFree(ctx->g1.log);
    if (ctx->g1.counters) (void) hipFree(ctx->g1.counters);
    if (ctx->g1.pair_flags) (void) hipFree(ctx->g1.pair_flags);
    for (auto cb : ctx->g1_carry)
        if (cb) (void) hipFree(cb);
    if (ctx->d_collect_n) (void) hipFree(ctx->d_collect_n);
    if (ctx->d_collect_rows) (void) hipFree(ctx->d_collect_rows);
    if (ctx->d_add_rows) (void) hipFree(ctx->d_add_rows);
    if (ctx->d_row_flags) (void) hipFree(ctx->d_row_flags);
    if (ctx->ev_producer) (void) hipEventDestroy(ctx->ev_producer);
    delete ctx;
}

static int batch_geometry(trew_hip_ctx *ctx, const trew_hip_batch *b, u32 *max_seg, u32 *max_len) {
    const int mode = ctx->p.mode;
    const int MINM = ctx->p.min_mer, MAXM = ctx->p.max_mer, SL = ctx->dp.slice_len;
    u32 maxlen = 0, ms = 0;
    auto unit_seg = [&](u32 n1, u32 n2) {
        u32 m = 0;
        if (mode == TREW_MODE_LONG && (int) n1 >= SL) m = (u32) SL + n1 % (u32) SL;
        for (int slot = 0; slot < mode_slots(mode); slot++) {
            const Segment sg = get_segment(mode, slot, n1, n2, MINM, MAXM, SL);
            if (sg.valid) m = std::max(m, sg.len);
        }
        return m;
    };
    if (b->lengths && !b->on_device) {
        const u32 two_min = (u32) (2 * MINM), four_min = (u32) (4 * MINM), four_max = (u32) (4 * MAXM);
        if (mode == TREW_MODE_PAIR) {
            for (u64 i = 0; i + 1 < b->n_reads; i += 2) {
                const u32 a = b->lengths[i], c = b->lengths[i + 1], hi = std::max(a, c), lo = std::min(a, c);
                maxlen = std::max(maxlen, hi);
                if (lo >= four_min) ms = std::max(ms, (hi + 1) / 2);
                if (lo >= two_min && lo < four_max) ms = std::max(ms, hi);
            }
        } else if (mode == TREW_MODE_SHORT) {
            for (u64 i = 0; i < b->n_reads; i++) {
                const u32 n = b->lengths[i];
                maxlen = std::max(maxlen, n);
                if (n >= two_min && n < four_max) ms = std::max(ms, n);
            }
            if (maxlen >= four_min) ms = std::max(ms, (maxlen + 1) / 2);
        } else if (mode == TREW_MODE_LONG) {
            for (u64 i = 0; i < b->n_reads; i++) {
                const u32 n = b->lengths[i];
                maxlen = std::max(maxlen, n);
                if ((int) n >= SL) ms = std::max(ms, (u32) SL + n % (u32) SL);
            }
        } else {
            for (u64 i = 0; i < b->n_reads; i++) {
                maxlen = std::max(maxlen, b->lengths[i]);
                ms = std::max(ms, unit_seg(b->lengths[i], 0));
            }
        }
    } else if (b->lengths) {
        maxlen = b->max_length > 0 ? (u32) b->max_length : (u32) kMaxSegBases;
        if (mode == TREW_MODE_SHORT || mode == TREW_MODE_PAIR)
            ms = std::max((maxlen + 1) / 2, std::min<u32>(maxlen, (u32) (4 * MAXM - 1)));
        else if (mode == TREW_MODE_LONG)
            ms = std::min<u32>(maxlen, (u32) (2 * SL - 1));
        else
            ms = maxlen;
    } else {
        maxlen = b->uniform_length;
        ms = unit_seg(maxlen, maxlen);
    }
    if ((mode == TREW_MODE_SHORT || mode == TREW_MODE_PAIR) && maxlen > 1000)
        return fail(ctx, "This mode is designed for short-read sequencing. Please use 'trew long'.");
    if (mode == TREW_MODE_SEGMENT && maxlen > (u32) kMaxSegBases) return fail(ctx, "segment longer than 1023 bases");
    *max_seg = ms;
    *max_len = maxlen;
    return 0;
}

struct BatchCopy {
    trew_hip_ctx *ctx;
    Slot &s;
    std::unique_lock<std::mutex> lk;
    BatchCopy(trew_hip_ctx *c, Slot &sl) : ctx(c), s(sl) {}
    int begin() {
        lk = std::unique_lock<std::mutex>(ctx->copy_mu);
        if (hipStreamQuery(s.stream) != hipSuccess) {
            (void) hipGetLastError();
            HIPCHK(ctx, hipEventRecord(s.ev_tail, s.stream));
            HIPCHK(ctx, hipStreamWaitEvent(ctx->copy_stream, s.ev_tail, 0));
        }
        return 0;
    }
    int copy(void *dst, const void *src, u64 bytes) {
        HIPCHK(ctx, hipMemcpyAsync(dst, src, bytes, hipMemcpyHostToDevice, ctx->copy_stream));
        return 0;
    }
// ... 47 lines not shown
            db->offsets = s.d_buf + b->n_words;
            db->lengths = s.d_buf + b->n_words + b->n_reads;
            return 0;
        }
        if (int rc = bc.copy(s.d_words, b->words, b->n_words * 4)) return rc;
        db->words = s.d_words;
        db->offsets = nullptr;
        db->lengths = nullptr;
        if (b->offsets) {
            if (int rc = bc.copy(s.d_offsets, b->offsets, b->n_reads * 4)) return rc;
            if (int rc = bc.copy(s.d_lengths, b->lengths, b->n_reads * 4)) return rc;
            db->offsets = s.d_offsets;
            db->lengths = s.d_lengths;
        }
        if (int rc = bc.end()) return rc;
    }
    return 0;
}

static int stage_thresholds(trew_hip_ctx *ctx, Slot &s, const DevBatch &db, const int2 **out) {
    *out = nullptr;
    if (db.offsets || db.lengths || db.uniform_length == 0) return 0;
    if (s.thr_length != db.uniform_length) {
        HIPCHK(ctx, hipStreamSynchronize(s.stream));
        fill_thresholds(ctx->dp, db.uniform_length, s.h_thr);
        HIPCHK(ctx, hipMemcpyAsync(s.d_thr, s.h_thr, kThrTableBytes, hipMemcpyHostToDevice, s.stream));
        s.thr_length = db.uniform_length;
    }
    *out = s.d_thr;
    return 0;
}

static int sync_all(trew_hip_ctx *ctx);

static int launch_batch(trew_hip_ctx *ctx, Slot &s, const DevBatch &db, u32 max_seg, u32 max_len) {
    s.n_units = db.n_units;
    if (db.n_units == 0) return 0;
    if (ctx->p.mode == TREW_MODE_SEGMENT) {
        HIPCHK(ctx, hipMemsetAsync(s.res.k_high, 0, db.n_reads * 4, s.stream));
        HIPCHK(ctx, hipMemsetAsync(s.res.k_low, 0, db.n_reads * 4, s.stream));
        HIPCHK(ctx, hipMemsetAsync(s.res.seq_high, 0, db.n_reads * 8, s.stream));
        HIPCHK(ctx, hipMemsetAsync(s.res.seq_low, 0, db.n_reads * 8, s.stream));
        HIPCHK(ctx, hipMemsetAsync(s.res.seq_high_hi, 0, db.n_reads * 8, s.stream));
        HIPCHK(ctx, hipMemsetAsync(s.res.seq_low_hi, 0, db.n_reads * 8, s.stream));
    }
    const u32 wl_cap = (u32) ctx->p.max_batch_reads;
    u32 *const wl_count = s.d_wl_count + (s.n_launches & 1) * kWlCountWords;
    u32 *const wl_count_next = s.d_wl_count + ((s.n_launches + 1) & 1) * kWlCountWords;
    auto submit_failed = [&](int rc) {
        const std::string keep = g_thread_error;
        (void) hipMemsetAsync(s.d_wl_count, 0, 2 * kWlCountBytes, s.stream);
        (void) hipStreamSynchronize(s.stream);
        g_thread_error = keep;
        return rc;
    };
#define SUBMIT_CHK(expr)                                                                       \
    do {                                                                                       \
        hipError_t e_ = (expr);                                                                \
        if (e_ != hipSuccess) {                                                                \
            g_thread_error = std::string(#expr) + ": " + hipGetErrorString(e_);               \
            return submit_failed((int) e_);                                                    \
        }                                                                                      \
    } while (0)
    const int2 *d_thr = nullptr;
    if (int rc = stage_thresholds(ctx, s, db, &d_thr)) return submit_failed(rc);
    const bool compat_g1 = (ctx->p.flags & TREW_FLAG_COMPAT_G1) != 0;
    if (compat_g1) SUBMIT_CHK(hipMemsetAsync(ctx->g1.pair_flags, 0, db.n_units, s.stream));
    const bool timed = !(ctx->p.flags & TREW_FLAG_NO_TIMING);
    hipEvent_t *ev = s.ev[s.n_submits % Slot::kRing];
    if (timed) SUBMIT_CHK(hipEventRecord(ev[0], s.stream));
    SUBMIT_CHK(launch_filter(s.stream, (u32) ctx->n_cu, max_seg, ctx->dp, db, s.d_wl, wl_count, wl_cap, nullptr, 0, ctx->table.overflow, d_thr));
    if (timed) SUBMIT_CHK(hipEventRecord(ev[1], s.stream));
    const u32 exact_seg = ctx->p.mode == TREW_MODE_LONG ? std::min<u32>(max_len, (u32) (2 * ctx->dp.slice_len - 1)) : max_len;
    const u32 cap = std::max<u32>(64u, ((exact_seg + 1 + 63u) / 64u) * 64u);
    const u32 rawwords = ctx->p.mode == TREW_MODE_LONG ? 4u : 3u * ((max_len + 31u) / 32u) + 1u;
    const int me = (int) (&s - ctx->slots.data());
    const int prev = ctx->last_slot.exchange(me, std::memory_order_relaxed);
    bool share = false;
    if (prev >= 0 && prev != me) {
        share = hipStreamQuery(ctx->slots[(size_t) prev].stream) == hipErrorNotReady;
        (void) hipGetLastError();
    }
    const bool with_bounds = s.d_bnd != nullptr && bounds_pass_applies(ctx->dp, max_seg);
    if (with_bounds) SUBMIT_CHK(launch_bounds(s.stream, (u32) ctx->n_cu, db.n_units, ctx->dp, db, s.d_wl, wl_count, wl_cap, s.d_bnd, s.bnd_cap));
    SUBMIT_CHK(launch_exact(s.stream, (u32) ctx->n_cu, db.n_units, ctx->dp, db, ctx->table_g1, s.d_wl, wl_count, wl_count_next, wl_cap, s.res, cap, rawwords, max_seg, share,
                            with_bounds ? s.d_bnd : nullptr, s.bnd_cap));
    if (timed) SUBMIT_CHK(hipEventRecord(ev[2], s.stream));
    if (compat_g1) {
        SUBMIT_CHK(launch_g1_apply(s.stream, ctx->table, ctx->g1, db, ctx->dp.min_mer, ctx->g1_carry[ctx->g1_batches & 1], ctx->g1_carry[(ctx->g1_batches + 1) & 1],
                                   ctx->g1_carry_cap));
        ctx->g1_batches++;
    }
#undef SUBMIT_CHK
    s.n_launches++;
    s.n_submits++;
    if (ctx->p.flags & TREW_FLAG_TRACK_PRESSURE)
        HIPCHK(ctx, hipMemcpyAsync(s.h_seen, ctx->table.overflow, kDiagWords * 4, hipMemcpyDeviceToHost, s.stream));
    return 0;
}

extern "C" int trew_hip_submit(trew_hip_ctx *ctx, const trew_hip_batch *batch, int slot) {
    if (!ctx || !batch) return -1;
    if (slot < 0 || slot >= (int) ctx->slots.size()) return fail(ctx, "slot out of range");
    HIPCHK(ctx, hipSetDevice(ctx->p.device));
    Slot &s = ctx->slots[(size_t) slot];
    u32 max_seg = 0, max_len = 0;
    if (int rc = batch_geometry(ctx, batch, &max_seg, &max_len)) return rc;
    DevBatch db;
    if (int rc = stage_batch(ctx, batch, s, &db)) return rc;
    return launch_batch(ctx, s, db, max_seg, max_len);
}

static int stage_ascii(trew_hip_ctx *ctx, const trew_hip_ascii_batch *a, Slot &s, DevBatch *db, u64 *n_words_out) {
    if (!s.d_ascii) return fail(ctx, "the context was created with max_batch_ascii_bytes = 0");
    if (a->n_reads > ctx->p.max_batch_reads) return fail(ctx, "batch has more reads than max_batch_reads");
    if (ctx->p.mode == TREW_MODE_PAIR && (a->n_reads & 1)) return fail(ctx, "pair mode needs an even number of reads");
    const bool ragged = a->word_offsets != nullptr;
    if (ragged != (a->byte_offsets != nullptr) || ragged != (a->lengths != nullptr)) return fail(ctx, "word_offsets, byte_offsets and lengths must all be given or all be NULL");
    u64 n_words = 0;
    if (ragged) {
        u64 w = 0;
        for (u64 i = 0; i < a->n_reads; i++) {
            if (a->word_offsets[i] != w) return fail(ctx, "word_offsets is not the running sum of the packed read sizes");
            if ((u64) a->byte_offsets[i] + a->lengths[i] > a->n_bytes) return fail(ctx, "a read's byte offset / length points outside the batch's bases");
            w += 3ull * (((u64) a->lengths[i] + 31ull) / 32ull);
            if (w > 0xffffffffull) return fail(ctx, "batch packs to more than 2^32 words");
        }
        n_words = w;
        if (a->n_bytes + 12ull * a->n_reads > ctx->p.max_batch_ascii_bytes) return fail(ctx, "text batch larger than max_batch_ascii_bytes");
    } else {
        if (a->uniform_length == 0 && a->n_reads) return fail(ctx, "uniform text batch without uniform_length");
        if (a->n_reads * (u64) a->uniform_length > a->n_bytes) return fail(ctx, "uniform text batch: n_reads * uniform_length exceeds n_bytes");
        if (a->n_bytes > ctx->p.max_batch_ascii_bytes) return fail(ctx, "text batch larger than max_batch_ascii_bytes");
        n_words = a->n_reads * 3ull * (((u64) a->uniform_length + 31ull) / 32ull);
    }
    if (n_words > ctx->p.max_batch_words) return fail(ctx, "batch has more words than max_batch_words");
    *n_words_out = n_words;
    db->n_reads = a->n_reads;
    db->n_units = ctx->p.mode == TREW_MODE_PAIR ? a->n_reads / 2 : a->n_reads;
    db->words = s.d_words;
    if (a->n_reads == 0) return 0;
    const unsigned char *d_bases;
    const u32 *d_wo = nullptr, *d_bo = nullptr, *d_len = nullptr;
    if (ragged) {
        u32 *arr = (u32 *) s.d_ascii;
        d_wo = arr;
        d_bo = arr + a->n_reads;
        d_len = arr + 2 * a->n_reads;
        d_bases = s.d_ascii + 12ull * a->n_reads;
        const bool one = a->byte_offsets == a->word_offsets + a->n_reads && a->lengths == a->byte_offsets + a->n_reads &&
                         (const void *) a->bases == (const void *) (a->lengths + a->n_reads);
        BatchCopy bc(ctx, s);
        if (int rc = bc.begin()) return rc;
        if (one) {
            if (int rc = bc.copy(s.d_ascii, a->word_offsets, 12ull * a->n_reads + a->n_bytes)) return rc;
        } else {
            if (int rc = bc.copy(arr, a->word_offsets, 4ull * a->n_reads)) return rc;
            if (int rc = bc.copy(arr + a->n_reads, a->byte_offsets, 4ull * a->n_reads)) return rc;
            if (int rc = bc.copy(arr + 2 * a->n_reads, a->lengths, 4ull * a->n_reads)) return rc;
            if (int rc = bc.copy(s.d_ascii + 12ull * a->n_reads, a->bases, a->n_bytes)) return rc;
        }
        if (int rc = bc.end()) return rc;
        db->offsets = d_wo;
        db->lengths = d_len;
        db->uniform_length = 0;
        db->uniform_stride = 0;
    } else {
        d_bases = s.d_ascii;
        BatchCopy bc(ctx, s);
// ... 136 lines not shown
                if (a.table != b.table) return a.table < b.table;
                if (a.k != b.k) return a.k < b.k;
                if (a.word_hi != b.word_hi) return a.word_hi < b.word_hi;
                return a.word_lo < b.word_lo;
            });
            u64 m = 0;
            for (u64 i = 0; i < n; i++) {
                if (m && rows[m - 1].table == rows[i].table && rows[m - 1].k == rows[i].k && rows[m - 1].word_hi == rows[i].word_hi &&
                    rows[m - 1].word_lo == rows[i].word_lo)
                    rows[m - 1].count += rows[i].count;
                else
                    rows[m++] = rows[i];
            }
            u64 z = 0;
            for (u64 i = 0; i < m; i++)
                if (rows[i].count) rows[z++] = rows[i];
            n = z;
        }
    }
    *n_rows = n;
    return 0;
}

extern "C" int trew_hip_collect_device(trew_hip_ctx *ctx, trew_hip_row *d_rows, uint64_t cap, uint64_t *n_rows) {
    if (!ctx || !n_rows) return -1;
    std::lock_guard<std::mutex> lk(ctx->table_mu);
    if (int rc = sync_all(ctx)) return rc;
    HIPCHK(ctx, hipDeviceSynchronize());
    return compact_to(ctx, -1, d_rows, d_rows ? cap : 0, n_rows);
}

extern "C" int trew_hip_collect_slice_device(trew_hip_ctx *ctx, trew_hip_row *d_slice, uint64_t slice_rows, void *consumer_stream, uint64_t *n_rows) {
    if (!ctx || !d_slice) return -1;
    std::lock_guard<std::mutex> lk(ctx->table_mu);
    if (int rc = sync_all(ctx)) return rc;
    hipStream_t st = ctx->slots[0].stream;
    if (consumer_stream) {
        HIPCHK(ctx, hipEventRecord(ctx->ev_producer, (hipStream_t) consumer_stream));
        HIPCHK(ctx, hipStreamWaitEvent(st, ctx->ev_producer, 0));
    } else {
        HIPCHK(ctx, hipDeviceSynchronize());
    }
    if (!ctx->d_collect_n) HIPCHK(ctx, hipMalloc((void **) &ctx->d_collect_n, 8));
    HIPCHK(ctx, hipMemsetAsync(ctx->d_collect_n, 0, 8, st));
    HIPCHK(ctx, launch_compact(st, ctx->table, ctx->table_slots, ctx->wide.wide_log2_slots, -1, d_slice + 1, slice_rows, ctx->d_collect_n));
    HIPCHK(ctx, launch_slice_finish(st, d_slice, slice_rows, ctx->d_collect_n, ctx->wide.spill_rows, ctx->wide.spill_n, ctx->wide.spill_cap));
    if (consumer_stream) {
        HIPCHK(ctx, hipEventRecord(ctx->ev_producer, st));
        HIPCHK(ctx, hipStreamWaitEvent((hipStream_t) consumer_stream, ctx->ev_producer, 0));
    }
    if (n_rows || !consumer_stream) {
        trew_hip_row h;
        memset(&h, 0, sizeof(h));
        HIPCHK(ctx, hipMemcpyAsync(&h, d_slice, sizeof(h), hipMemcpyDeviceToHost, st));
        HIPCHK(ctx, hipStreamSynchronize(st));
        if (n_rows) *n_rows = h.count;
    }
    return 0;
}

static int reset_locked(trew_hip_ctx *ctx) {
    hipStream_t fs = ctx->fill_stream;
    HIPCHK(ctx, hipMemsetAsync(ctx->table.keys, 0, ctx->table_slots * 8, fs));
    HIPCHK(ctx, hipMemsetAsync(ctx->table.counts, 0, ctx->table_slots * 8, fs));
    HIPCHK(ctx, hipMemsetAsync(ctx->table.overflow, 0, kDiagWords * 4, fs));
    const size_t wb = (size_t) 8 << ctx->wide.wide_log2_slots;
    HIPCHK(ctx, hipMemsetAsync(ctx->wide.wtag, 0, wb, fs));
    HIPCHK(ctx, hipMemsetAsync(ctx->wide.wlo, 0, wb, fs));
    HIPCHK(ctx, hipMemsetAsync(ctx->wide.whi, 0, wb, fs));
    HIPCHK(ctx, hipMemsetAsync(ctx->wide.wcount, 0, wb, fs));
    HIPCHK(ctx, fallback_counters_clear(fs));
    if (ctx->g1.counters) HIPCHK(ctx, hipMemsetAsync(ctx->g1.counters, 0, 16, fs));
    if (int rc = order_behind_fills(ctx)) return rc;
    std::lock_guard<std::mutex> lk(ctx->seen_mu);
    for (auto &sl : ctx->slots) memset(sl.h_seen, 0, kDiagWords * 4);
    for (auto &v : ctx->seen) v.store(0, std::memory_order_relaxed);
    return 0;
}

extern "C" int trew_hip_reset_tables(trew_hip_ctx *ctx) {
    if (!ctx) return -1;
    std::lock_guard<std::mutex> lk(ctx->table_mu);
    if (int rc = sync_all(ctx)) return rc;
    return reset_locked(ctx);
}

extern "C" int trew_hip_table_pressure(trew_hip_ctx *ctx, uint64_t *used_slots, uint64_t *total_slots, uint64_t *spilled_rows,
                                       uint64_t *spill_capacity) {
    if (!ctx) return -1;
    HIPCHK(ctx, hipSetDevice(ctx->p.device));
    u32 diag[kDiagWords];
    if (ctx->p.flags & TREW_FLAG_TRACK_PRESSURE) {
        std::lock_guard<std::mutex> lk(ctx->seen_mu);
        for (auto &sl : ctx->slots) {
            u32 copy[kDiagWords];
            for (int i = 0; i < kDiagWords; i++) copy[i] = ((volatile const u32 *) sl.h_seen)[i];
            note_seen(ctx, copy);
        }
        for (int i = 0; i < kDiagWords; i++) diag[i] = ctx->seen[i].load(std::memory_order_relaxed);
    } else {
        HIPCHK(ctx, hipStreamSynchronize(ctx->fill_stream));
        HIPCHK(ctx, hipMemcpy(diag, ctx->table.overflow, sizeof(diag), hipMemcpyDeviceToHost));
    }
    const u32 n_spill = diag[kDiagSpillRows];
    const u64 wide_slots = 1ull << ctx->wide.wide_log2_slots;
    const u64 wide_scaled = (u64) ((double) diag[kDiagInsertedWide] / (double) wide_slots * (double) ctx->table_slots);
    if (used_slots) *used_slots = std::max<u64>(diag[kDiagInserted], wide_scaled);
    if (total_slots) *total_slots = ctx->table_slots;
    if (spilled_rows) *spilled_rows = diag[kDiagOverflow] ? (u64) ctx->wide.spill_cap + 1 : n_spill;
    if (spill_capacity) *spill_capacity = ctx->wide.spill_cap;
    return 0;
}

static int add_device_rows_locked(trew_hip_ctx *ctx, const trew_hip_row *d_rows, u64 n_rows, bool validate) {
    hipStream_t st = ctx->slots[0].stream;
    if (validate) HIPCHK(ctx, hipMemsetAsync(ctx->d_row_flags, 0, kRowFlagWords * 4, st));
    HIPCHK(ctx, launch_add_rows(st, ctx->table, d_rows, n_rows, validate ? ctx->d_row_flags : nullptr));
    u32 flags[kRowFlagWords] = {0, 0, 0, 0};
    if (validate) HIPCHK(ctx, hipMemcpyAsync(flags, ctx->d_row_flags, sizeof(flags), hipMemcpyDeviceToHost, st));
    HIPCHK(ctx, hipStreamSynchronize(st));
    if (flags[kRowFlagBad]) return fail(ctx, "trew_hip_add_rows_device: row out of range (nothing was added)");
    u32 diag[kDiagWords];
    return check_diag(ctx, diag);
}

extern "C" int trew_hip_add_rows(trew_hip_ctx *ctx, const trew_hip_row *rows, uint64_t n_rows) {
    if (!ctx) return -1;
    if (n_rows == 0) return 0;
    for (u64 i = 0; i < n_rows; i++)
        if (rows[i].k < 1 || rows[i].k > 64 || rows[i].table < 0 || rows[i].table >= TREW_NUM_TABLES || (rows[i].k <= 32 && rows[i].word_hi))
            return fail(ctx, "trew_hip_add_rows: row out of range");
    std::lock_guard<std::mutex> lk(ctx->table_mu);
    if (int rc = sync_all(ctx)) return rc;
    if (int rc = ensure_rows(ctx, &ctx->d_add_rows, &ctx->add_cap, n_rows)) return rc;
    HIPCHK(ctx, hipMemcpyAsync(ctx->d_add_rows, rows, n_rows * sizeof(trew_hip_row), hipMemcpyHostToDevice, ctx->slots[0].stream));
    return add_device_rows_locked(ctx, ctx->d_add_rows, n_rows, false);
}

extern "C" int trew_hip_add_rows_device(trew_hip_ctx *ctx, const trew_hip_row *d_rows, uint64_t n_rows) {
    if (!ctx) return -1;
    if (n_rows == 0) return 0;
    if (!d_rows) return fail(ctx, "trew_hip_add_rows_device: null rows");
    std::lock_guard<std::mutex> lk(ctx->table_mu);
    if (int rc = sync_all(ctx)) return rc;
    HIPCHK(ctx, hipDeviceSynchronize());
    return add_device_rows_locked(ctx, d_rows, n_rows, true);
}

extern "C" int trew_hip_add_gathered_device(trew_hip_ctx *ctx, const trew_hip_row *d_buf, uint32_t n_slices, uint32_t own_slice,
                                            uint64_t slice_rows, void *producer_stream, uint64_t *max_rows) {
    if (!ctx) return -1;
    if (!d_buf || n_slices == 0 || own_slice >= n_slices) return fail(ctx, "trew_hip_add_gathered_device: bad arguments");
    std::lock_guard<std::mutex> lk(ctx->table_mu);
    if (int rc = sync_all(ctx)) return rc;
    hipStream_t st = ctx->slots[0].stream;
    if (producer_stream) {
        HIPCHK(ctx, hipEventRecord(ctx->ev_producer, (hipStream_t) producer_stream));
        HIPCHK(ctx, hipStreamWaitEvent(st, ctx->ev_producer, 0));
    } else {
        HIPCHK(ctx, hipDeviceSynchronize());
    }
    HIPCHK(ctx, hipMemsetAsync(ctx->d_row_flags, 0, kRowFlagWords * 4, st));
    HIPCHK(ctx, launch_add_gathered(st, ctx->table, d_buf, n_slices, own_slice, slice_rows, ctx->d_row_flags));
    u32 flags[kRowFlagWords] = {0, 0, 0, 0};
    HIPCHK(ctx, hipMemcpyAsync(flags, ctx->d_row_flags, sizeof(flags), hipMemcpyDeviceToHost, st));
    HIPCHK(ctx, hipStreamSynchronize(st));
    if (max_rows) *max_rows = ((u64) flags[kRowFlagMaxHi] << 32) | flags[kRowFlagMaxLo];
    if (flags[kRowFlagBad]) return fail(ctx, "trew_hip_add_gathered_device: row out of range (nothing was added)");
    if (flags[kRowFlagOverflow]) return 0;
    u32 diag[kDiagWords];
    return check_diag(ctx, diag);
}

extern "C" int trew_hip_debug_worklist(trew_hip_ctx *ctx, int slot, uint32_t *units, uint64_t cap, uint64_t *n) {
    if (!ctx || !n) return -1;
    if (slot < 0 || slot >= (int) ctx->slots.size()) return fail(ctx, "slot out of range");
    HIPCHK(ctx, hipSetDevice(ctx->p.device));
    Slot &s = ctx->slots[(size_t) slot];
    HIPCHK(ctx, hipStreamSynchronize(s.stream));
    u32 c = 0;
    if (s.n_launches) HIPCHK(ctx, hipMemcpy(&c, s.d_wl_count + ((s.n_launches - 1) & 1) * kWlCountWords, 4, hipMemcpyDeviceToHost));
    c = (u32) std::min<u64>(c, ctx->p.max_batch_reads);
    *n = c;
    const u64 take = std::min<u64>(c, cap);
    if (units && take) HIPCHK(ctx, hipMemcpy(units, s.d_wl, take * 4, hipMemcpyDeviceToHost));
    return 0;
}

extern "C" int trew_hip_debug_counters(trew_hip_ctx *ctx, uint64_t *out, int n) {
    if (!ctx || !out || n < 0) return -1;
    if (int rc = sync_all(ctx)) return rc;
    u32 diag[kDiagWords], fb[kFallbackWords];
    HIPCHK(ctx, hipMemcpy(diag, ctx->table.overflow, sizeof(diag), hipMemcpyDeviceToHost));
    HIPCHK(ctx, fallback_counters_read(fb));
    const u32 v[TREW_DEBUG_COUNTERS] = {fb[kFallbackStrictRerun], fb[kFallbackWindows], fb[kFallbackWideSpin], diag[kDiagInserted], diag[kDiagInsertedWide], fb[kFallbackGroupPunt], fb[kFallbackGroupRouted], fb[kFallbackGroupTarget], fb[kFallbackHalfDrain], fb[kFallbackUnitDrain]};
    for (int i = 0; i < n; i++) out[i] = i < TREW_DEBUG_COUNTERS ? v[i] : 0;
    return 0;
}

extern "C" int trew_hip_merge(trew_hip_ctx *dst, trew_hip_ctx *src) {
    if (!dst || !src) return -1;
    if (dst == src) return fail(dst, "trew_hip_merge: source and destination are the same context");
    std::mutex *m1 = &dst->table_mu, *m2 = &src->table_mu;
    if (m2 < m1) std::swap(m1, m2);
    std::lock_guard<std::mutex> l1(*m1), l2(*m2);
    if (int rc = sync_all(src)) return rc;
    u64 n = 0;
    if (int rc = compact_to(src, -1, nullptr, 0, &n)) return rc;
    if (n == 0) return 0;
    if (int rc = ensure_rows(src, &src->d_collect_rows, &src->collect_cap, n)) return rc;
    if (int rc = compact_to(src, -1, src->d_collect_rows, src->collect_cap, &n)) return rc;
    if (int rc = sync_all(dst)) return rc;
    if (int rc = ensure_rows(dst, &dst->d_add_rows, &dst->add_cap, n)) return rc;
    HIPCHK(dst, hipSetDevice(dst->p.device));
    HIPCHK(dst, hipMemcpyPeerAsync(dst->d_add_rows, dst->p.device, src->d_collect_rows, src->p.device, n * sizeof(trew_hip_row), dst->slots[0].stream));
    return add_device_rows_locked(dst, dst->d_add_rows, n, false);
}

extern "C" int trew_hip_segment_results(trew_hip_ctx *ctx, int slot, int32_t *k_high, int32_t *k_low,
                                        uint64_t *seq_high, uint64_t *seq_low, uint64_t *seq_high_hi, uint64_t *seq_low_hi,
                                        uint64_t n_reads) {
    if (!ctx) return -1;
    if (ctx->p.mode != TREW_MODE_SEGMENT) return fail(ctx, "segment results exist only in TREW_MODE_SEGMENT");
    if (slot < 0 || slot >= (int) ctx->slots.size()) return fail(ctx, "slot out of range");
    if (int rc = trew_hip_wait(ctx, slot)) return rc;
    Slot &s = ctx->slots[(size_t) slot];
    if (n_reads > s.n_units) return fail(ctx, "n_reads exceeds the last batch");
    if (k_high) HIPCHK(ctx, hipMemcpy(k_high, s.res.k_high, n_reads * 4, hipMemcpyDeviceToHost));
    if (k_low) HIPCHK(ctx, hipMemcpy(k_low, s.res.k_low, n_reads * 4, hipMemcpyDeviceToHost));
    if (seq_high) HIPCHK(ctx, hipMemcpy(seq_high, s.res.seq_high, n_reads * 8, hipMemcpyDeviceToHost));
    if (seq_low) HIPCHK(ctx, hipMemcpy(seq_low, s.res.seq_low, n_reads * 8, hipMemcpyDeviceToHost));
    if (seq_high_hi) HIPCHK(ctx, hipMemcpy(seq_high_hi, s.res.seq_high_hi, n_reads * 8, hipMemcpyDeviceToHost));
    if (seq_low_hi) HIPCHK(ctx, hipMemcpy(seq_low_hi, s.res.seq_low_hi, n_reads * 8, hipMemcpyDeviceToHost));
    return 0;
}

extern "C" int trew_hip_filter_masks(trew_hip_ctx *ctx, const trew_hip_batch *batch, uint64_t *cand, int slots_per_read) {
    if (!ctx || !batch || !cand) return -1;
    if (slots_per_read < 1 || slots_per_read > kMaxSlots) return fail(ctx, "slots_per_read out of range");
    if (int rc = sync_all(ctx)) return rc;
    Slot &s = ctx->slots[0];
    u32 max_seg = 0, max_len = 0;
    if (int rc = batch_geometry(ctx, batch, &max_seg, &max_len)) return rc;
    DevBatch db;
    if (int rc = stage_batch(ctx, batch, s, &db)) return rc;
    if (db.n_units == 0) return 0;
    u64 *d = nullptr;
    const u64 bytes = db.n_units * (u64) slots_per_read * 8ull;
    HIPCHK(ctx, hipMalloc((void **) &d, bytes));
    u32 *const wl_count = s.d_wl_count + (s.n_launches & 1) * kWlCountWords;
    const int2 *d_thr = nullptr;
    if (int rc = stage_thresholds(ctx, s, db, &d_thr)) {
        (void) hipFree(d);
        return rc;
    }
    hipError_t e = hipMemsetAsync(d, 0, bytes, s.stream);
    if (e == hipSuccess)
        e = launch_filter(s.stream, (u32) ctx->n_cu, max_seg, ctx->dp, db, s.d_wl, wl_count, (u32) ctx->p.max_batch_reads, d, slots_per_read,
                          ctx->table.overflow, d_thr);
    if (e == hipSuccess) e = hipMemsetAsync(wl_count, 0, kWlCountBytes, s.stream);
    if (e == hipSuccess) e = hipStreamSynchronize(s.stream);
    if (e == hipSuccess) e = hipMemcpy(cand, d, bytes, hipMemcpyDeviceToHost);
    (void) hipFree(d);
    HIPCHK(ctx, e);
    return 0;
}

extern "C" int trew_hip_last_timing(trew_hip_ctx *ctx, int slot, float *ms_filter, float *ms_exact, uint64_t *n_flagged) {
    if (!ctx) return -1;
    if (slot < 0 || slot >= (int) ctx->slots.size()) return fail(ctx, "slot out of range");
    if (ctx->p.flags & TREW_FLAG_NO_TIMING) return fail(ctx, "the context was created with TREW_FLAG_NO_TIMING");
    if (int rc = trew_hip_wait(ctx, slot)) return rc;
    Slot &s = ctx->slots[(size_t) slot];
    u64 first = s.n_reported;
    if (s.n_submits - first > (u64) Slot::kRing) first = s.n_submits - Slot::kRing;
    if (first == s.n_submits) return fail(ctx, "no timed submit on this slot since the last query");
    double sf = 0, se = 0;
    for (u64 i = first; i < s.n_submits; i++) {
// ... 876 lines not shown
```

### trew_amd/csrc/trew_common.hpp

```cpp
#pragma once
#include <stdint.h>

#include "../../include/trew_hip.h"

namespace trew {

typedef uint32_t u32;
typedef uint64_t u64;

constexpr int kMaxSlots = 6;
constexpr int kMaxSegBases = 1023;
constexpr int kTablePartBits = 9;
constexpr int kThrRows = kMaxSlots + 2;
constexpr int kThrJointRows = 4;
constexpr int kThrRow = 66;
constexpr size_t kThrTableBytes = (size_t) kThrRows * kThrRow * 8 + (size_t) kThrJointRows * kThrRow * 16;
constexpr int kThrNever = 1 << 20;

struct DevParams {
    int min_mer, max_mer;
    double low, high;
    float lowf;
    int slice_len;
    int mode;
    u32 flags;
};

struct DevBatch {
    const u32 *words;
    const u32 *offsets;
    const u32 *lengths;
    u32 uniform_length;
    u32 uniform_stride;
    u64 n_reads;
    u64 n_units;
};

constexpr int kChunkCounterWord = 16;

enum {
    kDiagOverflow = 0,
    kDiagWorklistDrop = 1,
    kDiagIntentDrop = 2,
    kDiagInserted = 3,
    kDiagInsertedWide = 4,
    kDiagKernarg = 5,
    kDiagSpillRows = 6,
    kDiagG1Drop = 7,
    kDiagWords = 16
};

enum {
    kFallbackStrictRerun = 0,
    kFallbackWindows = 1,
    kFallbackWideSpin = 2,
    kFallbackGroupPunt = 3,
    kFallbackGroupRouted = 4,
    kFallbackGroupTarget = 5,
    kFallbackHalfDrain = 6,
    kFallbackUnitDrain = 7,
    kFallbackWords = 8
};

enum { kRowFlagBad = 0, kRowFlagOverflow = 1, kRowFlagMaxLo = 2, kRowFlagMaxHi = 3, kRowFlagWords = 4 };

struct DevTable {
    u64 *keys;
    u64 *counts;
    u32 log2_part_slots;
    u32 *overflow;
    const struct DevWide *wide;
};

struct DevG1 {
    trew_hip_row *log;
    u32 *counters;
    unsigned char *pair_flags;
    u32 log_cap;
};


struct DevWide {
    u64 *wtag, *wlo, *whi, *wcount;
    u32 wide_log2_slots;
    u32 spill_cap;
    trew_hip_row *spill_rows;
    u32 *spill_n;
    u32 spin_limit;
};

struct DevTableG1 {
    DevTable t;
    DevG1 g;
    DevWide w;
};

struct SegResults {
    int32_t *k_high;
    int32_t *k_low;
    u64 *seq_high;
    u64 *seq_low;
    u64 *seq_high_hi;
    u64 *seq_low_hi;
};

constexpr int kAnnotMaxMotifs = TREW_ANNOT_MAX_MOTIFS;
struct AnnotMotifDev {
    u32 k;
    u32 pad[3];
    u32 plo[2][32];
    u32 phi[2][32];
};

struct IntervalRulesDev {
    u32 max_gap[kAnnotMaxMotifs], min_len[kAnnotMaxMotifs];
};
struct IntervalLog {
    unsigned long long *counter;
    u32 *recs;
    u64 cap;
};
// ... 137 lines not shown
```

### trew_amd/csrc/trew_kernels.hip

```cpp
#include <hip/hip_runtime.h>

#include <algorithm>
#include <cstdlib>

#include "trew_common.hpp"
#include "trew_launch.hpp"
#include "trew_synth.hpp"

#ifndef TREW_FILTER_THREADS
#define TREW_FILTER_THREADS 256
#endif

namespace trew {

typedef unsigned __int128 u128;

#include "kernels/helpers.inc"
#include "kernels/bound.inc"
#include "kernels/prefilter.inc"
#include "kernels/count_table.inc"
#include "kernels/exact_core.inc"
#include "kernels/decide_group.inc"
#include "kernels/bounds_pass.inc"
#include "kernels/driver_long.inc"
// ... 42 lines not shown
                const volatile float prod = (float) W * P.lowf;
                const int Weff = uni_windows(nw, (int) sg.len, k);
                th.x = (int) floorf(prod) + 1 - (W - Weff);
                th.y = Weff - th.x;
            }
            table[slot * kThrRow + k - 1] = th;
        }
    }
    for (int p = 0; p < 2; p++) {
        const Segment a = get_segment(P.mode, 2 * p, uniform_length, uniform_length, P.min_mer, P.max_mer, P.slice_len);
        const Segment b = get_segment(P.mode, 2 * p + 1, uniform_length, uniform_length, P.min_mer, P.max_mer, P.slice_len);
        const bool ok = 2 * p + 1 < nslots && a.valid && b.valid && b.len == a.len + 1;
        for (int k = 1; k <= kThrRow; k++) {
            int2 th;
            th.x = kThrNever;
            th.y = -1;
            const int WA = (int) a.len - k + 1, WB = WA + 1;
            if (ok && WA > 0) {
                const int Weff = uni_windows(nw, (int) a.len, k);
                const volatile float pa = (float) WA * P.lowf, pb = (float) WB * P.lowf;
                const int xa = (int) floorf(pa) + 1 - (WA - Weff), xb = (int) floorf(pb) + 1 - (WB - Weff);
                th.x = std::min(xa, xb);
                th.y = Weff - th.x;
            }
            table[(kMaxSlots + p) * kThrRow + k - 1] = th;
        }
    }
    int4 *joint = (int4 *) (table + kThrRows * kThrRow);
    for (int r = 0; r < kThrJointRows; r++) {
        const int2 *src = table + (r < 2 ? 2 * r : kMaxSlots + (r - 2)) * kThrRow;
        for (int k = 1; k <= kThrRow; k++) {
            const int2 th = src[k - 1];
            joint[r * kThrRow + k - 1] = make_int4(-2 * th.x, -th.x, 3 * th.x - th.y - 1, th.x);
        }
    }
}

hipError_t launch_filter(hipStream_t st, u32 n_cu, u32 max_seg_len, const DevParams &P, const DevBatch &B, u32 *wl, u32 *wl_count,
                         u32 wl_cap, u64 *dbg_masks, int dbg_slots, u32 *diag, const int2 *d_thr) {
    const int nw = pick_nw(max_seg_len);
    const int max_seg = (int) std::min<u32>(max_seg_len, (u32) (32 * nw - 1));
    if (B.n_units == 0) return hipSuccess;
    typedef void (*kern_t)(DevParams, DevBatch, u32 *, u32 *, u32, u64 *, int, int, u32 *, const int2 *);
    const kern_t fn = nw == 3 ? filter_kernel<3> : nw == 5 ? filter_kernel<5> : nw == 10 ? filter_kernel<10> : filter_kernel<32>;
    const u32 threads = kFilterThreads;
    static thread_local kern_t cached_fn = nullptr;
    static thread_local int cached_per_cu = 0;
    int per_cu = cached_per_cu;
    if (cached_fn != fn) {
        if (hipOccupancyMaxActiveBlocksPerMultiprocessor(&per_cu, (const void *) fn, (int) threads, 0) != hipSuccess || per_cu < 1) per_cu = 4;
        if (const char *e = getenv("TREW_FILTER_BLOCKS_PER_CU")) per_cu = std::max(1, atoi(e));
        cached_fn = fn;
        cached_per_cu = per_cu;
    }
    u64 blocks = (B.n_units + threads - 1) / threads;
    const u64 persistent = (u64) n_cu * (u64) per_cu;
    if (blocks > persistent) blocks = persistent;
    hipLaunchKernelGGL(fn, dim3((u32) blocks), dim3(threads), 0, st, P, B, wl, wl_count, wl_cap, dbg_masks, dbg_slots, max_seg, diag, d_thr);
    return hipGetLastError();
}

hipError_t fallback_counters_read(u32 *out) { return hipMemcpyFromSymbol(out, HIP_SYMBOL(g_fallback), sizeof(u32) * kFallbackWords); }
hipError_t fallback_counters_clear(hipStream_t st) {
    void *p = nullptr;
    const hipError_t e = hipGetSymbolAddress(&p, HIP_SYMBOL(g_fallback));
    return e != hipSuccess ? e : hipMemsetAsync(p, 0, sizeof(u32) * kFallbackWords, st);
}

u32 exact_lds_bytes_host(u32 cap, u32 rawwords, u32 wordbytes) { return exact_lds_bytes(cap, rawwords, wordbytes); }

hipError_t launch_g1_apply(hipStream_t st, const DevTable &T, const DevG1 &G, const DevBatch &B, int min_mer, const trew_hip_row *carry_in,
                           trew_hip_row *carry_out, u32 carry_cap) {
    hipLaunchKernelGGL(g1_apply_kernel, dim3(256), dim3(256), 0, st, T, G, B, min_mer, carry_in, carry_out, carry_cap);
    hipLaunchKernelGGL(g1_finish_kernel, dim3(1), dim3(1), 0, st, G);
    return hipGetLastError();
}

bool bounds_pass_applies(const DevParams &P, u32 max_seg_len) {
    return P.mode == TREW_MODE_SHORT && P.max_mer <= 32 && !(P.flags & TREW_FLAG_NO_FILTER) && pick_nw(max_seg_len) == 3 &&
           P.max_mer - P.min_mer < (int) kBoundWords && !(P.flags & TREW_FLAG_DEBUG_NO_GROUP);
}
size_t bounds_entry_bytes() { return kBoundItemWords * sizeof(u32); }

hipError_t launch_bounds(hipStream_t st, u32 n_cu, u64 n_units, const DevParams &P, const DevBatch &B, const u32 *wl, const u32 *wl_count,
                         u32 wl_cap, u32 *bnd, u32 bnd_cap) {
    if (n_units == 0 || bnd_cap == 0) return hipSuccess;
    const u64 most = (std::min<u64>(n_units, bnd_cap) * 2 + 63) / 64;
    const u32 grid = (u32) std::min<u64>((u64) n_cu * 16ull, most);
    hipLaunchKernelGGL(bounds_kernel<3>, dim3(grid), dim3(64), 0, st, P, B, wl, wl_count, wl_cap, bnd, bnd_cap);
    return hipGetLastError();
}

hipError_t launch_exact(hipStream_t st, u32 n_cu, u64 n_units, const DevParams &P, const DevBatch &B, const DevTableG1 &T,
                        const u32 *wl, u32 *wl_count, u32 *wl_count_next, u32 wl_cap, const SegResults &R, u32 cap, u32 rawwords,
                        u32 max_seg_len, bool share, const u32 *bnd, u32 bnd_cap) {
    const bool wide = P.max_mer > 32;
    const u32 lds = exact_lds_bytes(cap, rawwords, wide ? 16u : 8u);
    const u32 bound_len = P.mode == TREW_MODE_LONG ? (u32) P.slice_len : max_seg_len;
    const int nw = (P.flags & TREW_FLAG_NO_FILTER) ? 0 : pick_nw(bound_len);
    typedef void (*kern_t)(DevParams, DevBatch, DevTableG1, const u32 *, u32 *, u32 *, u32, SegResults, u32, u32, const u32 *, u32);
    kern_t fn = nullptr;
    if (!bounds_pass_applies(P, max_seg_len)) bnd = nullptr;
#define TREW_PICK_MODE(NWV, WTV)                                                      \
    switch (P.mode) {                                                                 \
    case TREW_MODE_SHORT: fn = exact_kernel<NWV, TREW_MODE_SHORT, WTV>; break;        \
    case TREW_MODE_PAIR: fn = exact_kernel<NWV, TREW_MODE_PAIR, WTV>; break;          \
    case TREW_MODE_LONG: fn = exact_kernel<NWV, TREW_MODE_LONG, WTV>; break;          \
    default: fn = exact_kernel<NWV, TREW_MODE_SEGMENT, WTV>; break;                   \
    }
    if (!wide) {
        switch (nw) {
        case 3: TREW_PICK_MODE(3, u64) break;
        case 5: TREW_PICK_MODE(5, u64) break;
        case 10: TREW_PICK_MODE(10, u64) break;
        default: TREW_PICK_MODE(0, u64) break;
        }
    } else {
        switch (nw) {
        case 3: TREW_PICK_MODE(3, u128) break;
        case 5: TREW_PICK_MODE(5, u128) break;
        case 10: TREW_PICK_MODE(10, u128) break;
        default: TREW_PICK_MODE(0, u128) break;
        }
    }
#undef TREW_PICK_MODE
    static thread_local kern_t cached_fn = nullptr;
    static thread_local u32 cached_lds = 0;
    static thread_local int cached_per_cu = 0;
    int per_cu = 8;
    if (cached_fn == fn && cached_lds == lds) {
        per_cu = cached_per_cu;
    } else {
        if (hipOccupancyMaxActiveBlocksPerMultiprocessor(&per_cu, (const void *) fn, 64, lds) != hipSuccess || per_cu < 1) per_cu = 8;
        cached_fn = fn;
        cached_lds = lds;
        cached_per_cu = per_cu;
    }
    per_cu = per_cu > 32 ? 32 : per_cu;
    if (share && P.mode == TREW_MODE_SHORT) per_cu = std::max(1, per_cu / 2);
    if (const char *e = getenv("TREW_EXACT_WAVES_PER_CU")) per_cu = std::max(1, atoi(e));
    const u64 full = (u64) n_cu * (u64) per_cu;
    const u32 grid = (u32) std::min<u64>(full, std::max<u64>(n_units / 16, 64));
    hipLaunchKernelGGL(fn, dim3(grid), dim3(64), lds, st, P, B, T, wl, wl_count, wl_count_next, wl_cap, R, cap, rawwords, bnd, bnd ? bnd_cap : 0u);
    return hipGetLastError();
}

hipError_t launch_add_rows(hipStream_t st, const DevTable &T, const trew_hip_row *d_rows, u64 n, u32 *d_flags) {
    if (n == 0) return hipSuccess;
    const dim3 grid((u32) ((n + 255) / 256));
    if (d_flags) hipLaunchKernelGGL(table_check_rows_kernel, grid, dim3(256), 0, st, d_rows, n, d_flags);
    hipLaunchKernelGGL(table_add_rows_kernel, grid, dim3(256), 0, st, T, d_rows, n, (const u32 *) d_flags);
    return hipGetLastError();
}

hipError_t launch_add_gathered(hipStream_t st, const DevTable &T, const trew_hip_row *d_buf, u32 n_slices, u32 own, u64 slice_rows, u32 *d_flags) {
    const u64 total = (u64) n_slices * (slice_rows + 1ull);
    if (total == 0) return hipSuccess;
    const dim3 grid((u32) ((total + 255) / 256));
    hipLaunchKernelGGL(table_check_gathered_kernel, grid, dim3(256), 0, st, d_buf, n_slices, own, slice_rows, d_flags);
    hipLaunchKernelGGL(table_add_gathered_kernel, grid, dim3(256), 0, st, T, d_buf, n_slices, own, slice_rows, (const u32 *) d_flags);
    return hipGetLastError();
}

hipError_t launch_pack_ascii(hipStream_t st, const unsigned char *d_bases, const u32 *d_byte_offsets, const u32 *d_lengths, const u32 *d_word_offsets,
                             u32 uniform_length, u64 n_reads, u64 n_triples, u32 *d_words) {
    if (n_triples == 0) return hipSuccess;
    hipLaunchKernelGGL(pack_ascii_kernel, dim3((u32) ((n_triples + 255) / 256)), dim3(256), 0, st, d_bases, d_byte_offsets, d_lengths, d_word_offsets, uniform_length,
                       n_reads, n_triples, d_words);
    return hipGetLastError();
}

hipError_t launch_compact(hipStream_t st, const DevTable &T, u64 n_slots, u32 wide_log2_slots, int table, trew_hip_row *d_rows, u64 cap,
                          unsigned long long *d_n) {
    const u64 total = n_slots + (1ull << wide_log2_slots);
    hipLaunchKernelGGL(table_compact_kernel, dim3((u32) ((total + 255) / 256)), dim3(256), 0, st, T, n_slots, table, d_rows, cap, d_n);
    return hipGetLastError();
}

hipError_t launch_slice_finish(hipStream_t st, trew_hip_row *d_slice, u64 slice_rows, const unsigned long long *d_n, const trew_hip_row *d_spill_rows,
                               const u32 *d_spill_n, u32 spill_cap) {
    hipLaunchKernelGGL(table_slice_finish_kernel, dim3((spill_cap + 255u) / 256u), dim3(256), 0, st, d_slice, slice_rows, d_n, d_spill_rows, d_spill_n, spill_cap);
    return hipGetLastError();
}

hipError_t launch_annotate(hipStream_t st, u32 n_cu, const DevBatch &B, const AnnotMotifDev *d_motifs, int n_motifs, u32 max_len, bool general,
                           trew_hip_annot *d_out) {
    if (B.n_reads == 0) return hipSuccess;
    if (general || max_len > 256u) {
        const u64 blocks = std::min<u64>((B.n_reads + 3ull) / 4ull, (u64) n_cu * 8ull);
        hipLaunchKernelGGL(annotate_wave_kernel, dim3((u32) blocks), dim3(256), 0, st, B, d_motifs, n_motifs, (u32 *) d_out);
    } else {
        const dim3 grid((u32) ((B.n_reads + 255ull) / 256ull));
        if (max_len <= 160u)
            hipLaunchKernelGGL(annotate_lane_kernel<5>, grid, dim3(256), 0, st, B, d_motifs, n_motifs, (uint2 *) d_out);
        else
            hipLaunchKernelGGL(annotate_lane_kernel<8>, grid, dim3(256), 0, st, B, d_motifs, n_motifs, (uint2 *) d_out);
    }
    return hipGetLastError();
}

hipError_t launch_tracts(hipStream_t st, u32 n_cu, const DevBatch &B, const AnnotMotifDev *d_motifs, int n_motifs, int penalty, trew_hip_tract *d_out) {
    if (B.n_reads == 0) return hipSuccess;
    const u64 blocks = std::min<u64>((B.n_reads + 3ull) / 4ull, (u64) n_cu * 8ull);
    hipLaunchKernelGGL(tracts_wave_kernel, dim3((u32) blocks), dim3(256), 0, st, B, d_motifs, n_motifs, penalty, (u32 *) d_out);
    return hipGetLastError();
}

hipError_t launch_intervals(hipStream_t st, u32 n_cu, const DevBatch &B, const AnnotMotifDev *d_motifs, int n_motifs, const IntervalRulesDev &rules,
                            const IntervalLog &lg, u32 *d_counts) {
    if (B.n_reads == 0) return hipSuccess;
    const u64 blocks = std::min<u64>((B.n_reads + 3ull) / 4ull, (u64) n_cu * 8ull);
    hipLaunchKernelGGL(intervals_wave_kernel, dim3((u32) blocks), dim3(256), 0, st, B, d_motifs, n_motifs, rules, lg, d_counts);
    return hipGetLastError();
}

hipError_t launch_variants(hipStream_t st, u32 n_cu, const DevBatch &B, const AnnotMotifDev *d_motifs, int n_motifs, trew_hip_variant *d_out,
                           unsigned long long *d_hist, unsigned long long *d_reads_with) {
    if (B.n_reads == 0) return hipSuccess;
    const u64 blocks = std::min<u64>((B.n_reads + 3ull) / 4ull, (u64) n_cu * 8ull);
    hipLaunchKernelGGL(variants_wave_kernel, dim3((u32) blocks), dim3(256), 0, st, B, d_motifs, n_motifs, (u32 *) d_out, d_hist, d_reads_with);
    return hipGetLastError();
}

hipError_t launch_periods(hipStream_t st, u32 n_cu, const DevBatch &B, int min_period, int max_period, int penalty, u32 min_score, trew_hip_period *d_out) {
    if (B.n_reads == 0) return hipSuccess;
    const u64 blocks = std::min<u64>((B.n_reads + 3ull) / 4ull, (u64) n_cu * 8ull);
// ... 87 lines not shown
```

### trew_amd/csrc/trew_launch.hpp

```cpp
#pragma once
#include <hip/hip_runtime.h>

#include "trew_common.hpp"

namespace trew {

int pick_nw(u32 max_seg_len);

hipError_t launch_filter(hipStream_t st, u32 n_cu, u32 max_seg_len, const DevParams &P, const DevBatch &B, u32 *wl, u32 *wl_count,
                         u32 wl_cap, u64 *dbg_masks, int dbg_slots, u32 *diag, const int2 *d_thr);
void fill_thresholds(const DevParams &P, u32 uniform_length, int2 *table);
hipError_t launch_exact(hipStream_t st, u32 n_cu, u64 n_units, const DevParams &P, const DevBatch &B, const DevTableG1 &T,
                        const u32 *wl, u32 *wl_count, u32 *wl_count_next, u32 wl_cap, const SegResults &R, u32 cap, u32 rawwords,
                        u32 max_seg_len, bool share, const u32 *bnd, u32 bnd_cap);
bool bounds_pass_applies(const DevParams &P, u32 max_seg_len);
size_t bounds_entry_bytes();
hipError_t launch_bounds(hipStream_t st, u32 n_cu, u64 n_units, const DevParams &P, const DevBatch &B, const u32 *wl, const u32 *wl_count,
                         u32 wl_cap, u32 *bnd, u32 bnd_cap);
u32 exact_lds_bytes_host(u32 cap, u32 rawwords, u32 wordbytes);
hipError_t launch_g1_apply(hipStream_t st, const DevTable &T, const DevG1 &G, const DevBatch &B, int min_mer, const trew_hip_row *carry_in,
                           trew_hip_row *carry_out, u32 carry_cap);
hipError_t fallback_counters_read(u32 *out);
hipError_t fallback_counters_clear(hipStream_t st);
hipError_t launch_add_rows(hipStream_t st, const DevTable &T, const trew_hip_row *d_rows, u64 n, u32 *d_flags);
hipError_t launch_add_gathered(hipStream_t st, const DevTable &T, const trew_hip_row *d_buf, u32 n_slices, u32 own, u64 slice_rows, u32 *d_flags);
hipError_t launch_pack_ascii(hipStream_t st, const unsigned char *d_bases, const u32 *d_byte_offsets, const u32 *d_lengths, const u32 *d_word_offsets,
                             u32 uniform_length, u64 n_reads, u64 n_triples, u32 *d_words);
hipError_t launch_compact(hipStream_t st, const DevTable &T, u64 n_slots, u32 wide_log2_slots, int table, trew_hip_row *d_rows, u64 cap,
                          unsigned long long *d_n);
hipError_t launch_slice_finish(hipStream_t st, trew_hip_row *d_slice, u64 slice_rows, const unsigned long long *d_n, const trew_hip_row *d_spill_rows,
                               const u32 *d_spill_n, u32 spill_cap);
hipError_t launch_annotate(hipStream_t st, u32 n_cu, const DevBatch &B, const AnnotMotifDev *d_motifs, int n_motifs, u32 max_len, bool general,
                           trew_hip_annot *d_out);
hipError_t launch_tracts(hipStream_t st, u32 n_cu, const DevBatch &B, const AnnotMotifDev *d_motifs, int n_motifs, int penalty, trew_hip_tract *d_out);
hipError_t launch_intervals(hipStream_t st, u32 n_cu, const DevBatch &B, const AnnotMotifDev *d_motifs, int n_motifs, const IntervalRulesDev &rules,
                            const IntervalLog &lg, u32 *d_counts);
hipError_t launch_variants(hipStream_t st, u32 n_cu, const DevBatch &B, const AnnotMotifDev *d_motifs, int n_motifs, trew_hip_variant *d_out,
                           unsigned long long *d_hist, unsigned long long *d_reads_with);
hipError_t launch_periods(hipStream_t st, u32 n_cu, const DevBatch &B, int min_period, int max_period, int penalty, u32 min_score, trew_hip_period *d_out);
hipError_t launch_chain(hipStream_t st, u32 n_cu, const DevBatch &B, const AnnotMotifDev *d_motifs, int n_motifs, const ChainLog &lg, u32 *d_counts);
hipError_t launch_repeats(hipStream_t st, u32 n_cu, const DevBatch &B, int min_period, int max_period, int penalty, u32 min_score, const RepeatLog &lg,
                          u32 *d_counts);
hipError_t launch_satellites(hipStream_t st, u32 n_cu, const DevBatch &B, int min_period, int max_period, int penalty, u32 min_score,
                             const RepeatLog &lg, u32 *d_counts);
hipError_t launch_align(hipStream_t st, u32 n_cu, const DevBatch &B, const AnnotMotifDev *d_motifs, int n_motifs, int penalty, trew_hip_alignment *d_out);
hipError_t launch_trace(hipStream_t st, u32 n_cu, const DevBatch &B, const AnnotMotifDev *d_motifs, int n_motifs, int penalty, u32 min_score,
                        const TraceLog &lg, trew_hip_alignment *d_out, u32 *d_counts);
hipError_t launch_decompose(hipStream_t st, u32 n_cu, const DevBatch &B, int min_period, int max_period, int penalty, u32 min_score, const TraceLog &lg,
                            trew_hip_refined *d_out, u32 *d_counts);
hipError_t launch_refine(hipStream_t st, u32 n_cu, const DevBatch &B, int min_period, int max_period, int penalty, u32 min_score, trew_hip_refined *d_out);
hipError_t launch_tandems(hipStream_t st, u32 n_cu, const DevBatch &B, int min_period, int max_period, int penalty, u32 min_score, const RepeatLog &lg,
                          u32 *d_counts);
hipError_t launch_synth_short(hipStream_t st, u64 seed, u64 first, u64 n, u32 len, u32 *d_words);
hipError_t launch_synth_long(hipStream_t st, u64 seed, u64 first, u64 n, const u32 *d_qtable, const u32 *d_offsets, u32 *d_words);
hipError_t launch_synth_pair(hipStream_t st, u64 seed, u64 first, u64 n, u32 len, u32 *d_words);

}
```

Before: 2115.

## Compact bounds pass into a live list and sharpen N-containing bounds

The bounds kernel now compacts its output so that only reads whose halves may still pass the thresholds are written to a live list. The exact kernel then iterates over that list instead of the full worklist, and dead reads are counted. It also computes a sharper 16-bucket bound using an adjacency feature for segments containing N, replaces the double-precision threshold test with an integer lookup table held in LDS, and moves to 4-wave blocks with a block-level prefix via atomics. This adds atomics, block syncs and a debug flag and API in exchange for skipping exact work on reads that cannot pass.

```diff
diff --git a/include/trew_hip.h b/include/trew_hip.h
--- a/include/trew_hip.h
+++ b/include/trew_hip.h
@@ -40,6 +40,7 @@
     TREW_FLAG_DEBUG_NO_GROUP = 1024,
     TREW_FLAG_DEBUG_ANNOT_GENERAL = 8192,
     TREW_FLAG_DEBUG_SMALL_BOUNDS = 16384,
+    TREW_FLAG_DEBUG_NO_LIVE_LIST = 32768,
     TREW_FLAG_TRACK_PRESSURE = 256
 };
 
@@ -115,10 +116,12 @@
 int trew_hip_table_pressure(trew_hip_ctx *ctx, uint64_t *used_slots, uint64_t *total_slots, uint64_t *spilled_rows,
                             uint64_t *spill_capacity);
 
-#define TREW_DEBUG_COUNTERS 10
+#define TREW_DEBUG_COUNTERS 11
 int trew_hip_debug_counters(trew_hip_ctx *ctx, uint64_t *out, int n);
 
 int trew_hip_debug_worklist(trew_hip_ctx *ctx, int slot, uint32_t *units, uint64_t cap, uint64_t *n);
+
+int trew_hip_debug_live_list(trew_hip_ctx *ctx, int slot, uint32_t *units, uint64_t cap, uint64_t *n);
 
 int trew_hip_segment_results(trew_hip_ctx *ctx, int slot, int32_t *k_high, int32_t *k_low,
                              uint64_t *seq_high, uint64_t *seq_low, uint64_t *seq_high_hi, uint64_t *seq_low_hi,
diff --git a/trew_amd/__init__.py b/trew_amd/__init__.py
--- a/trew_amd/__init__.py
+++ b/trew_amd/__init__.py
@@ -10,6 +10,7 @@
     FLAG_DEBUG_NO_JOINT,
     FLAG_DEBUG_NO_UNI_DRAIN,
     FLAG_DEBUG_SMALL_BOUNDS,
+    FLAG_DEBUG_NO_LIVE_LIST,
     FLAG_DEBUG_WIDE_NO_WAIT,
     MODE_LONG,
     MODE_PAIR,
diff --git a/trew_amd/capi.py b/trew_amd/capi.py
--- a/trew_amd/capi.py
+++ b/trew_amd/capi.py
@@ -19,6 +19,7 @@
 FLAG_DEBUG_NO_GROUP = 1024
 FLAG_DEBUG_ANNOT_GENERAL = 8192
 FLAG_DEBUG_SMALL_BOUNDS = 16384
+FLAG_DEBUG_NO_LIVE_LIST = 32768
 FLAG_DEBUG_WIDE_NO_WAIT = 128
 TABLE_NAMES = ("forward_high", "forward_low", "backward_high", "backward_low", "both_high", "both_low")
 
@@ -31,7 +32,7 @@
     "trew_pack_pairs", "trew_hip_host_alloc", "trew_hip_host_free", "trew_hip_device_count",
     "trew_synth_long_lengths", "trew_synth_long_ascii", "trew_synth_long_device",
     "trew_hip_collect_device", "trew_hip_add_rows_device", "trew_hip_merge", "trew_hip_table_pressure",
-    "trew_hip_add_gathered_device", "trew_hip_collect_slice_device", "trew_hip_debug_counters", "trew_hip_debug_worklist", "trew_hip_submit_ascii", "trew_hip_pack_ascii",
+    "trew_hip_add_gathered_device", "trew_hip_collect_slice_device", "trew_hip_debug_counters", "trew_hip_debug_worklist", "trew_hip_debug_live_list", "trew_hip_submit_ascii", "trew_hip_pack_ascii",
     "trew_motif_parse", "trew_hip_annotate", "trew_hip_annotate_results", "trew_annotate_host",
     "trew_hip_tracts", "trew_hip_tracts_results", "trew_tracts_host",
     "trew_hip_intervals", "trew_hip_intervals_results", "trew_intervals_host",
@@ -47,7 +48,7 @@
     "trew_hip_decompose", "trew_hip_decompose_results", "trew_decompose_host",
 )
 DEBUG_COUNTERS = ("strict_rerun", "windows_fallback", "wide_spin_timeout", "inserted", "inserted_wide", "group_punt", "group_routed", "group_target",
-                  "half_drain", "unit_drain")
+                  "half_drain", "unit_drain", "dead_entries")
 
 
 class Params(C.Structure):
@@ -248,6 +249,7 @@
     lib.trew_hip_collect_slice_device.argtypes = [vp, vp, u64, vp, C.POINTER(u64)]
     lib.trew_hip_debug_counters.argtypes = [vp, C.POINTER(u64), i32]
     lib.trew_hip_debug_worklist.argtypes = [vp, i32, vp, u64, C.POINTER(u64)]
+    lib.trew_hip_debug_live_list.argtypes = [vp, i32, vp, u64, C.POINTER(u64)]
     lib.trew_hip_table_pressure.argtypes = [vp, C.POINTER(u64), C.POINTER(u64), C.POINTER(u64), C.POINTER(u64)]
     lib.trew_hip_segment_results.argtypes = [vp, i32, vp, vp, vp, vp, vp, vp, u64]
     lib.trew_hip_filter_masks.argtypes = [vp, C.POINTER(Batch), vp, i32]
@@ -1007,13 +1009,19 @@
         self._chk(self.lib.trew_hip_debug_counters(self.ctx, out, len(DEBUG_COUNTERS)), "trew_hip_debug_counters")
         return dict(zip(DEBUG_COUNTERS, (int(x) for x in out)))
 
-    def debug_worklist(self, slot=0):
+    def _debug_units(self, fn, name, slot):
         n = C.c_uint64(0)
-        self._chk(self.lib.trew_hip_debug_worklist(self.ctx, slot, None, 0, C.byref(n)), "trew_hip_debug_worklist")
+        self._chk(fn(self.ctx, slot, None, 0, C.byref(n)), name)
         out = np.zeros(int(n.value), dtype=np.uint32)
         if len(out):
-            self._chk(self.lib.trew_hip_debug_worklist(self.ctx, slot, out.ctypes.data, len(out), C.byref(n)), "trew_hip_debug_worklist")
+            self._chk(fn(self.ctx, slot, out.ctypes.data, len(out), C.byref(n)), name)
         return out
+
+    def debug_worklist(self, slot=0):
+        return self._debug_units(self.lib.trew_hip_debug_worklist, "trew_hip_debug_worklist", slot)
+
+    def debug_live_list(self, slot=0):
+        return self._debug_units(self.lib.trew_hip_debug_live_list, "trew_hip_debug_live_list", slot)
 
     def merge_from(self, other):
         self._chk(self.lib.trew_hip_merge(self.ctx, other.ctx), "trew_hip_merge")
diff --git a/trew_amd/csrc/kernels/bound.inc b/trew_amd/csrc/kernels/bound.inc
--- a/trew_amd/csrc/kernels/bound.inc
+++ b/trew_amd/csrc/kernels/bound.inc
@@ -159,3 +159,49 @@
     }
     return links;
 }
+
+
+template <int NW>
+__device__ __forceinline__ void adjacency_parity(const u32 (&lo)[NW], const u32 (&hi)[NW], const u32 (&v1)[NW], u32 (&PD)[NW]) {
+    u32 D[NW];
+#pragma unroll
+    for (int j = 0; j < NW; j++) {
+        const int jn = j + 1 < NW ? j + 1 : 0;
+        const u32 nlo = alignbit(j + 1 < NW ? lo[jn] : 0u, lo[j], 1u), nhi = alignbit(j + 1 < NW ? hi[jn] : 0u, hi[j], 1u);
+        const u32 nv = alignbit(j + 1 < NW ? v1[jn] : 0u, v1[j], 1u);
+        D[j] = ~((lo[j] ^ nlo) | (hi[j] ^ nhi)) & v1[j] & nv;
+    }
+    prefix_parity<NW>(D, PD);
+}
+
+template <int NW>
+__device__ __forceinline__ u32 adjacency_feature_word(const u32 (&PD)[NW], const u32 (&lo)[NW], const u32 (&hi)[NW], int j, u32 s) {
+    const int jn = j + 1 < NW ? j + 1 : 0;
+    const u32 pd = alignbit(j + 1 < NW ? PD[jn] : 0u, PD[j], s);
+    const u32 sl = alignbit(j + 1 < NW ? lo[jn] : 0u, lo[j], s), sh = alignbit(j + 1 < NW ? hi[jn] : 0u, hi[j], s);
+    return PD[j] ^ pd ^ ~((lo[j] ^ sl) | (hi[j] ^ sh));
+}
+
+template <int N>
+__device__ __forceinline__ u32 max_bucket16(const u32 (&F1)[N], const u32 (&F2)[N], const u32 (&F3)[N], const u32 (&F4)[N], const u32 (&V)[N]) {
+    u32 c[16];
+#pragma unroll
+    for (int b = 0; b < 16; b++) c[b] = 0;
+#pragma unroll
+    for (int j = 0; j < N; j++) {
+        const u32 a[4] = {V[j] & ~(F1[j] | F2[j]), ~F1[j] & F2[j], F1[j] & ~F2[j], F1[j] & F2[j]};
+#pragma unroll
+        for (int q = 0; q < 4; q++) {
+            const u32 b1 = a[q] & F3[j], b0 = a[q] ^ b1;
+            const u32 d11 = b1 & F4[j], d01 = b0 & F4[j];
+            c[4 * q + 0] += __popc(b0 ^ d01);
+            c[4 * q + 1] += __popc(d01);
+            c[4 * q + 2] += __popc(b1 ^ d11);
+            c[4 * q + 3] += __popc(d11);
+        }
+    }
+    u32 m = 0;
+#pragma unroll
+    for (int b = 0; b < 16; b++) m = max(m, c[b]);
+    return m;
+}
diff --git a/trew_amd/csrc/kernels/bounds_pass.inc b/trew_amd/csrc/kernels/bounds_pass.inc
--- a/trew_amd/csrc/kernels/bounds_pass.inc
+++ b/trew_amd/csrc/kernels/bounds_pass.inc
@@ -1,51 +1,89 @@
 
 constexpr u32 kBoundsTileStride = kBoundWords + 1;
 
-__device__ __forceinline__ u32 pack_bound_word(u32 m8, u32 count, u32 links, u32 has_n, int k, int gmax, const DevParams &P) {
+__device__ __forceinline__ u32 pack_bound_word(u32 m8, u32 count, u32 links, u32 has_n, int k, int gmax, const DevParams &P, const u32 *need) {
     const u32 runs = count - links < 127u ? count - links : 127u;
-    const double dm = (double) m8, dc = (double) count;
-    const double tl = P.low * dc, th = P.high * dc;
-    u32 pass_lo = dm > tl ? 1u : 0u, pass_hi = dm > th ? 1u : 0u;
-    const bool amb = fabs(dm - tl) <= 1e-9 || fabs(dm - th) <= 1e-9;
-    if (__any(amb)) {
-        const double ub = count ? dm / dc : 0.0;
-        pass_lo = ub >= P.low ? 1u : 0u;
-        pass_hi = ub >= P.high ? 1u : 0u;
+    u32 pass_lo, pass_hi;
+    if (need) {
+        const u32 nd = need[count];
+        pass_lo = m8 >= (nd & 0xffffu) ? 1u : 0u;
+        pass_hi = m8 >= (nd >> 16) ? 1u : 0u;
+    } else {
+        const double dm = (double) m8, dc = (double) count;
+        const double tl = P.low * dc, th = P.high * dc;
+        pass_lo = dm > tl ? 1u : 0u, pass_hi = dm > th ? 1u : 0u;
+        const bool amb = fabs(dm - tl) <= 1e-9 || fabs(dm - th) <= 1e-9;
+        if (__any(amb)) {
+            const double ub = count ? dm / dc : 0.0;
+            pass_lo = ub >= P.low ? 1u : 0u;
+            pass_hi = ub >= P.high ? 1u : 0u;
+        }
     }
     const bool inr = k <= gmax && count != 0u;
     return inr ? (m8 | (count << 10) | (runs << 20) | (pass_lo << 27) | (pass_hi << 28) | (has_n << 29)) : (has_n << 29);
 }
 
+template <int N>
+__device__ __forceinline__ u32 sharpen_bound_word(u32 word, const u32 (&F1)[N], const u32 (&F2)[N], const u32 (&F3)[N], const u32 (&F4)[N],
+                                                  const u32 (&V)[N], u32 links, u32 has_n, int k, int gmax, const DevParams &P, const u32 *need) {
+    const u32 m8 = word & 1023u, count = (word >> 10) & 1023u;
+    const u32 m16 = max_bucket16<N>(F1, F2, F3, F4, V);
+    const u32 sharp = pack_bound_word(m16 < m8 ? m16 : m8, count, links, has_n, k, gmax, P, need);
+    return (has_n != 0u && (word & (3u << 27)) != 0u) ? sharp : word;
+}
+
+constexpr u32 kBoundsWaves = 4;
 template <int NW>
-__global__ __launch_bounds__(64) void bounds_kernel(DevParams P, DevBatch B, const u32 *__restrict__ wl, const u32 *__restrict__ wl_count, u32 wl_cap,
-                                                    u32 *__restrict__ bnd, u32 bnd_cap) {
+__global__ __launch_bounds__(64 * kBoundsWaves) void bounds_kernel(DevParams P, DevBatch B, const u32 *__restrict__ wl, u32 *__restrict__ wl_count,
+                                                                     u32 wl_cap, u32 *__restrict__ bnd, u32 bnd_cap, u32 *__restrict__ live,
+                                                                     const u32 *__restrict__ need_table) {
     static_assert(NW == 3, "the k loop is written for three words: halves of at most 95 bases");
-    __shared__ u32 tile[64 * kBoundsTileStride];
-    const u32 lane = lane_id();
+    __shared__ u32 tile_all[kBoundsWaves * 64 * kBoundsTileStride];
+    __shared__ u32 src_row_all[kBoundsWaves * 64];
+    __shared__ u32 wave_live[kBoundsWaves + 1];
+    const u32 lane = lane_id(), wave = threadIdx.x >> 6;
+    u32 *const tile = tile_all + wave * 64u * kBoundsTileStride;
+    u32 *const src_row = src_row_all + wave * 64u;
+    const bool sharpen = live != nullptr;
+    __shared__ u32 need_lds[kBoundNeedWords];
+    const u32 *const need = need_table ? need_lds : nullptr;
+    if (need_table) {
+        for (u32 i = threadIdx.x; i < (u32) kBoundNeedWords; i += 64u * kBoundsWaves) need_lds[i] = need_table[i];
+        __syncthreads();
+    }
     u32 n = wl_count[0];
     n = n < wl_cap ? n : wl_cap;
     n = n < bnd_cap ? n : bnd_cap;
+    if (!live && blockIdx.x == 0 && threadIdx.x == 0) wl_count[kStoredPrefixWord] = n;
     const u64 total = 2ull * n;
     const int klo = P.min_mer, khi = P.max_mer < P.min_mer + (int) kBoundWords - 1 ? P.max_mer : P.min_mer + (int) kBoundWords - 1;
-    for (u64 base = (u64) blockIdx.x * 64u; base < total; base += (u64) gridDim.x * 64u) {
-        const u64 idx = base + lane;
+    constexpr u32 kBlockHalves = 64u * kBoundsWaves;
+    for (u64 bbase = (u64) blockIdx.x * kBlockHalves; bbase < total; bbase += (u64) gridDim.x * kBlockHalves) {
+        const u64 idx = bbase + threadIdx.x;
         const bool active = idx < total;
         const u32 half = (u32) idx & 1u;
         ReadRef rd;
         rd.w = B.words;
         rd.len = rd.nw = 0;
-        if (active) rd = get_read(B, wl[idx >> 1]);
+        u32 unit = 0;
+        if (active) {
+            unit = wl[idx >> 1];
+            rd = get_read(B, unit);
+        }
         const Segment sg = get_segment(TREW_MODE_SHORT, (int) half, rd.len, 0, P.min_mer, P.max_mer, P.slice_len);
         const bool can = active && sg.valid && sg.len <= 32u * NW - 1u;
+        const bool whole = get_segment(TREW_MODE_SHORT, 2, rd.len, 0, P.min_mer, P.max_mer, P.slice_len).valid;
         if (!can) rd.nw = 0;
         const int L = can ? (int) sg.len : 0;
-        u32 lo[3], hi[3], nm[3], V[3], P1[3], P2[3], P3[3];
+        u32 lo[3], hi[3], nm[3], V[3], P1[3], P2[3], P3[3], PD[3];
         load_planes<3>(rd, sg.start, lo, hi, nm);
         segment_setup<3, false, true, true>(lo, hi, nm, L, V, P1, P2, P3);
+        adjacency_parity<3>(lo, hi, V, PD);
         const u32 has_n = segment_has_n<3>(nm, L) != 0u ? 1u : 0u;
         for (int t = 1; t < klo; t++) drain_v_step3(V);
         const int Lmax = (int) wave_max_u32((u32) L);
         u32 *const row = tile + lane * kBoundsTileStride;
+        u32 seen = 0;
         int k = klo;
         for (const int b = khi < Lmax - 64 ? khi : Lmax - 64; k <= b; k++) {
             const u32 bs = (u32) k;
@@ -60,7 +98,16 @@
             }
             const u32 count = bcnt_acc(V[2], bcnt_acc(V[1], __popc(V[0])));
             const u32 m8 = max_bucket8<3>(F1, F2, F3, V, count);
-            row[k - klo] = pack_bound_word(m8, count, class_links<3>(V, E), has_n, k, P.max_mer, P);
+            const u32 links = class_links<3>(V, E);
+            u32 word = pack_bound_word(m8, count, links, has_n, k, P.max_mer, P, need);
+            if (sharpen && __any(has_n != 0u && (word & (3u << 27)) != 0u)) {
+                u32 F4[3];
+#pragma unroll
+                for (int j = 0; j < 3; j++) F4[j] = adjacency_feature_word<3>(PD, lo, hi, j, bs - 1u);
+                word = sharpen_bound_word<3>(word, F1, F2, F3, F4, V, links, has_n, k, P.max_mer, P, need);
+            }
+            row[k - klo] = word;
+            seen |= word;
             drain_v_step3(V);
         }
         if (k <= khi) {
@@ -77,20 +124,48 @@
                 const u32 E[2] = {~((lo[0] ^ (u32) Sl) | (hi[0] ^ (u32) Sh)), ~((lo[1] ^ (u32) (Sl >> 32)) | (hi[1] ^ (u32) (Sh >> 32)))};
                 const u32 count = bcnt_acc(Vw[1], __popc(Vw[0]));
                 const u32 m8 = max_bucket8<2>(F1, F2, F3, Vw, count);
-                row[k - klo] = pack_bound_word(m8, count, class_links<2>(Vw, E), has_n, k, P.max_mer, P);
+                const u32 links = class_links<2>(Vw, E);
+                u32 word = pack_bound_word(m8, count, links, has_n, k, P.max_mer, P, need);
+                if (sharpen && __any(has_n != 0u && (word & (3u << 27)) != 0u)) {
+                    const u32 F4[2] = {adjacency_feature_word<3>(PD, lo, hi, 0, (u32) k - 1u), adjacency_feature_word<3>(PD, lo, hi, 1, (u32) k - 1u)};
+                    word = sharpen_bound_word<2>(word, F1, F2, F3, F4, Vw, links, has_n, k, P.max_mer, P, need);
+                }
+                row[k - klo] = word;
+                seen |= word;
                 Vq &= Vq >> 1;
             }
         }
         for (int ki = khi >= klo ? khi - klo + 1 : 0; ki < (int) kBoundWords; ki++) row[ki] = has_n << 29;
+        const u64 even = 0x5555555555555555ull;
+        const u64 activeb = __ballot(active);
+        const u64 dropb = __ballot(sharpen && can && !whole && (seen & (3u << 27)) == 0u);
+        const u64 liveb = activeb & ~(dropb & (dropb >> 1)) & even;
+        const u32 nlive = (u32) __popcll(liveb), nent = (u32) __popcll(activeb & even);
+        if (lane == 0) wave_live[wave] = nlive | (nent << 16);
+        __syncthreads();
+        if (live && threadIdx.x == 0) {
+            u32 tl = 0, te = 0;
+            for (u32 w = 0; w < kBoundsWaves; w++) tl += wave_live[w] & 0xffffu, te += wave_live[w] >> 16;
+            wave_live[kBoundsWaves] = atomicAdd(&wl_count[kStoredPrefixWord], tl);
+            if (te != tl) atomicAdd(&wl_count[kDeadEntriesWord], te - tl);
+        }
+        if (live) __syncthreads();
+        u32 pos0 = live ? wave_live[kBoundsWaves] : (u32) (bbase >> 1);
+        for (u32 w = 0; w < wave; w++) pos0 += wave_live[w] & 0xffffu;
+        const u32 mine = lane & ~1u;
+        if ((liveb >> mine) & 1ull) {
+            const u32 rank = (u32) __popcll(liveb & ((1ull << mine) - 1ull));
+            src_row[rank * 2u + half] = lane;
+            if (live && half == 0u) live[pos0 + rank] = unit;
+        }
         lds_sync();
-        const u64 left = total - base;
-        const u32 words = (left < 64u ? (u32) left : 64u) * kBoundWords;
-        u32 *const dst = bnd + base * kBoundWords;
+        const u32 words = nlive * 2u * kBoundWords;
+        u32 *const dst = bnd + (u64) pos0 * kBoundItemWords;
 #pragma unroll 4
         for (u32 r = 0; r < kBoundWords; r++) {
             const u32 w = r * 64u + lane;
-            if (w < words) dst[w] = tile[(w >> 5) * kBoundsTileStride + (w & 31u)];
+            if (w < words) dst[w] = tile[src_row[w >> 5] * kBoundsTileStride + (w & 31u)];
         }
-        lds_sync();
+        __syncthreads();
     }
 }
diff --git a/trew_amd/csrc/kernels/decide_group.inc b/trew_amd/csrc/kernels/decide_group.inc
--- a/trew_amd/csrc/kernels/decide_group.inc
+++ b/trew_amd/csrc/kernels/decide_group.inc
@@ -508,6 +508,7 @@
     u32 cap, rawwords;
     const u32 *bnd;
     u32 bnd_cap;
+    const u32 *live;
 };
 template <int NW, typename WT, typename SB>
 __device__ void run_short_group(ExactSmem sm, const DevParams &P, TableRef T, const ReadRef rdA, const ReadRef rdB, bool haveB, const SB sb) {
@@ -521,7 +522,7 @@
         typedef const __attribute__((address_space(4))) u64 *c64;
         typedef const __attribute__((address_space(4))) u32 *c32;
         const u64 ka = (u64) __builtin_amdgcn_kernarg_segment_ptr();
-        const u32 bcap = *(c32) (ka + offsetof(ExactKernArgs, bnd_cap));
+        const u32 bcap = *(c32) (*(c64) (ka + offsetof(ExactKernArgs, wl_count)) + 4u * kStoredPrefixWord);
         const u32 posA = rfl(sb.posA), posB = rfl(sb.posB);
         stored = posA < bcap && posB < bcap;
         if (stored && (lane < 32u || haveB)) {
diff --git a/trew_amd/csrc/kernels/exact_kernel.inc b/trew_amd/csrc/kernels/exact_kernel.inc
--- a/trew_amd/csrc/kernels/exact_kernel.inc
+++ b/trew_amd/csrc/kernels/exact_kernel.inc
@@ -18,7 +18,7 @@
 template <int NW, int MODE, typename WT>
 __global__ __launch_bounds__(64, (exact_waves<NW, MODE>(sizeof(WT) == 8))) void exact_kernel(DevParams P, DevBatch B, DevTableG1 TG, const u32 *wl,
                                                    u32 *wl_count, u32 *wl_count_next, u32 wl_cap, SegResults R, u32 cap, u32 rawwords,
-                                                   const u32 *bnd, u32 bnd_cap) {
+                                                   const u32 *bnd, u32 bnd_cap, const u32 *live) {
     typedef ExactKernArgs KernArgs;
     static_assert(alignof(DevParams) == 8 && alignof(DevBatch) == 8 && alignof(DevTableG1) == 8, "kernarg layout: 8-byte aligned argument structs");
     static_assert(sizeof(DevParams) % 8 == 0 && sizeof(DevBatch) % 8 == 0, "kernarg layout: no padding between the argument structs");
@@ -40,6 +40,8 @@
     sm.rw = nullptr;
     u32 n = wl_count[0];
     n = n < wl_cap ? n : wl_cap;
+    constexpr bool kLive = MODE == TREW_MODE_SHORT && NW == 3 && sizeof(WT) == 8;
+    if constexpr (kLive) n = wl_count[kStoredPrefixWord] + (n > bnd_cap ? n - bnd_cap : 0u);
 #ifdef TREW_PHASE_PROFILE
     if (lane_id() < 32) ph_lds()[lane_id()] = 0;
     __syncthreads();
@@ -91,7 +93,16 @@
         };
         auto chunk_items = [&](u64 w0l) __attribute__((always_inline)) -> u32 { return (u32) ((w0l + kUnits < n ? w0l + kUnits : n) - w0l); };
         auto fetch_units = [&](u32 bf, u64 w0l, u32 nit) __attribute__((always_inline)) {
-            if (lane < nit) __builtin_amdgcn_global_load_lds(wl + w0l + lane, (__attribute__((address_space(3))) u32 *) (meta_base + bf * kMetaWords), 4, 0, 0);
+            const u32 *src = wl + w0l + lane;
+            if constexpr (kLive) {
+                typedef const __attribute__((address_space(4))) u64 *c64;
+                typedef const __attribute__((address_space(4))) u32 *c32;
+                const u64 ka = (u64) __builtin_amdgcn_kernarg_segment_ptr();
+                const u32 pre = *(c32) (*(c64) (ka + offsetof(KernArgs, wl_count)) + 4u * kStoredPrefixWord);
+                const u32 p = (u32) w0l + lane;
+                src = p < pre ? (const u32 *) *(c64) (ka + offsetof(KernArgs, live)) + p : wl + (p - pre) + *(c32) (ka + offsetof(KernArgs, bnd_cap));
+            }
+            if (lane < nit) __builtin_amdgcn_global_load_lds(src, (__attribute__((address_space(3))) u32 *) (meta_base + bf * kMetaWords), 4, 0, 0);
         };
         auto fetch_words = [&](u32 bf, u32 nit) __attribute__((always_inline)) {
             typedef const __attribute__((address_space(4))) u64 *c64;
diff --git a/trew_amd/csrc/trew_capi.cpp b/trew_amd/csrc/trew_capi.cpp
--- a/trew_amd/csrc/trew_capi.cpp
+++ b/trew_amd/csrc/trew_capi.cpp
@@ -53,6 +53,8 @@
     u32 *d_wl_count = nullptr;
     u32 *d_bnd = nullptr;
     u32 bnd_cap = 0;
+    u32 *d_live = nullptr;
+    bool live_launch = false;
     int2 *d_thr = nullptr;
     int2 *h_thr = nullptr;
     hipEvent_t ev_tail = nullptr, ev_copied = nullptr;
@@ -104,6 +106,8 @@
     std::mutex table_mu;
     std::atomic<u32> seen[kDiagWords];
     std::atomic<int> last_slot{-1};
+    u32 *d_bound_need = nullptr;
+    std::atomic<int> dead_slot{-1};
     std::mutex seen_mu;
 };
 
@@ -279,6 +283,13 @@
     }
 
     if ((e = hipMalloc((void **) &ctx->d_row_flags, kRowFlagWords * 4)) != hipSuccess) return bail("hipMalloc(row flags)", e);
+    if (bounds_pass_applies(ctx->dp, 1)) {
+        u32 need[kBoundNeedWords];
+        if (fill_bound_needs(ctx->dp, need)) {
+            if ((e = hipMalloc((void **) &ctx->d_bound_need, sizeof(need))) != hipSuccess) return bail("hipMalloc(bound thresholds)", e);
+            if ((e = hipMemcpy(ctx->d_bound_need, need, sizeof(need), hipMemcpyHostToDevice)) != hipSuccess) return bail("hipMemcpy(bound thresholds)", e);
+        }
+    }
     if ((e = hipEventCreateWithFlags(&ctx->ev_producer, hipEventDisableTiming)) != hipSuccess) return bail("hipEventCreate", e);
     ctx->slots.resize((size_t) p.n_slots);
     for (auto &s : ctx->slots) {
@@ -306,6 +317,8 @@
             const u64 share = std::min<u64>(std::max<u64>(p.max_batch_reads / 32, std::min<u64>(p.max_batch_reads, 1ull << 16)), 1ull << 22);
             s.bnd_cap = (p.flags & TREW_FLAG_DEBUG_SMALL_BOUNDS) ? 64u : (u32) share;
             if ((e = hipMalloc((void **) &s.d_bnd, (size_t) s.bnd_cap * bounds_entry_bytes())) != hipSuccess) return bail("hipMalloc(bounds)", e);
+            if (!(p.flags & TREW_FLAG_DEBUG_NO_LIVE_LIST) && (e = hipMalloc((void **) &s.d_live, (size_t) s.bnd_cap * sizeof(u32))) != hipSuccess)
+                return bail("hipMalloc(live worklist)", e);
         }
         if ((e = hipMalloc((void **) &s.d_wl_count, 2 * kWlCountBytes)) != hipSuccess) return bail("hipMalloc(wl_count)", e);
         if ((e = hipMemsetAsync(s.d_wl_count, 0, 2 * kWlCountBytes, ctx->fill_stream)) != hipSuccess) return bail("hipMemsetAsync", e);
@@ -341,6 +354,7 @@
         if (s.h_thr) (void) hipHostFree(s.h_thr);
         if (s.d_wl) (void) hipFree(s.d_wl);
         if (s.d_bnd) (void) hipFree(s.d_bnd);
+        if (s.d_live) (void) hipFree(s.d_live);
         if (s.d_wl_count) (void) hipFree(s.d_wl_count);
         if (s.res.k_high) (void) hipFree(s.res.k_high);
         if (s.res.k_low) (void) hipFree(s.res.k_low);
@@ -384,6 +398,7 @@
     if (ctx->d_collect_rows) (void) hipFree(ctx->d_collect_rows);
     if (ctx->d_add_rows) (void) hipFree(ctx->d_add_rows);
     if (ctx->d_row_flags) (void) hipFree(ctx->d_row_flags);
+    if (ctx->d_bound_need) (void) hipFree(ctx->d_bound_need);
     if (ctx->ev_producer) (void) hipEventDestroy(ctx->ev_producer);
     delete ctx;
 }
@@ -597,9 +612,11 @@
         (void) hipGetLastError();
     }
     const bool with_bounds = s.d_bnd != nullptr && bounds_pass_applies(ctx->dp, max_seg);
-    if (with_bounds) SUBMIT_CHK(launch_bounds(s.stream, (u32) ctx->n_cu, db.n_units, ctx->dp, db, s.d_wl, wl_count, wl_cap, s.d_bnd, s.bnd_cap));
+    if (with_bounds) SUBMIT_CHK(launch_bounds(s.stream, (u32) ctx->n_cu, db.n_units, ctx->dp, db, s.d_wl, wl_count, wl_cap, s.d_bnd, s.bnd_cap, s.d_live, ctx->d_bound_need));
     SUBMIT_CHK(launch_exact(s.stream, (u32) ctx->n_cu, db.n_units, ctx->dp, db, ctx->table_g1, s.d_wl, wl_count, wl_count_next, wl_cap, s.res, cap, rawwords, max_seg, share,
-                            with_bounds ? s.d_bnd : nullptr, s.bnd_cap));
+                            with_bounds ? s.d_bnd : nullptr, s.bnd_cap, with_bounds ? s.d_live : nullptr));
+    s.live_launch = with_bounds && s.d_live != nullptr;
+    ctx->dead_slot.store(s.live_launch ? me : -1, std::memory_order_relaxed);
     if (timed) SUBMIT_CHK(hipEventRecord(ev[2], s.stream));
     if (compat_g1) {
         SUBMIT_CHK(launch_g1_apply(s.stream, ctx->table, ctx->g1, db, ctx->dp.min_mer, ctx->g1_carry[ctx->g1_batches & 1], ctx->g1_carry[(ctx->g1_batches + 1) & 1],
@@ -902,6 +919,7 @@
     if (!ctx) return -1;
     std::lock_guard<std::mutex> lk(ctx->table_mu);
     if (int rc = sync_all(ctx)) return rc;
+    ctx->dead_slot.store(-1, std::memory_order_relaxed);
     return reset_locked(ctx);
 }
 
@@ -1007,13 +1025,37 @@
     return 0;
 }
 
+extern "C" int trew_hip_debug_live_list(trew_hip_ctx *ctx, int slot, uint32_t *units, uint64_t cap, uint64_t *n) {
+    if (!ctx || !n) return -1;
+    if (slot < 0 || slot >= (int) ctx->slots.size()) return fail(ctx, "slot out of range");
+    HIPCHK(ctx, hipSetDevice(ctx->p.device));
+    Slot &s = ctx->slots[(size_t) slot];
+    if (!s.live_launch) return trew_hip_debug_worklist(ctx, slot, units, cap, n);
+    HIPCHK(ctx, hipStreamSynchronize(s.stream));
+    u32 blk[3] = {0, 0, 0};
+    HIPCHK(ctx, hipMemcpy(blk, s.d_wl_count + ((s.n_launches - 1) & 1) * kWlCountWords, sizeof(blk), hipMemcpyDeviceToHost));
+    const u64 flagged = std::min<u64>(blk[0], ctx->p.max_batch_reads);
+    const u64 pre = std::min<u64>(blk[kStoredPrefixWord], s.bnd_cap), tail = flagged > s.bnd_cap ? flagged - s.bnd_cap : 0;
+    *n = pre + tail;
+    const u64 take_pre = std::min<u64>(pre, cap), take_tail = std::min<u64>(tail, cap - take_pre);
+    if (units && take_pre) HIPCHK(ctx, hipMemcpy(units, s.d_live, take_pre * 4, hipMemcpyDeviceToHost));
+    if (units && take_tail) HIPCHK(ctx, hipMemcpy(units + take_pre, s.d_wl + s.bnd_cap, take_tail * 4, hipMemcpyDeviceToHost));
+    return 0;
+}
+
 extern "C" int trew_hip_debug_counters(trew_hip_ctx *ctx, uint64_t *out, int n) {
     if (!ctx || !out || n < 0) return -1;
     if (int rc = sync_all(ctx)) return rc;
     u32 diag[kDiagWords], fb[kFallbackWords];
     HIPCHK(ctx, hipMemcpy(diag, ctx->table.overflow, sizeof(diag), hipMemcpyDeviceToHost));
     HIPCHK(ctx, fallback_counters_read(fb));
-    const u32 v[TREW_DEBUG_COUNTERS] = {fb[kFallbackStrictRerun], fb[kFallbackWindows], fb[kFallbackWideSpin], diag[kDiagInserted], diag[kDiagInsertedWide], fb[kFallbackGroupPunt], fb[kFallbackGroupRouted], fb[kFallbackGroupTarget], fb[kFallbackHalfDrain], fb[kFallbackUnitDrain]};
+    u32 dead = 0;
+    const int ds = ctx->dead_slot.load(std::memory_order_relaxed);
+    if (ds >= 0) {
+        const Slot &s = ctx->slots[(size_t) ds];
+        if (s.n_launches) HIPCHK(ctx, hipMemcpy(&dead, s.d_wl_count + ((s.n_launches - 1) & 1) * kWlCountWords + kDeadEntriesWord, 4, hipMemcpyDeviceToHost));
+    }
+    const u32 v[TREW_DEBUG_COUNTERS] = {fb[kFallbackStrictRerun], fb[kFallbackWindows], fb[kFallbackWideSpin], diag[kDiagInserted], diag[kDiagInsertedWide], fb[kFallbackGroupPunt], fb[kFallbackGroupRouted], fb[kFallbackGroupTarget], fb[kFallbackHalfDrain], fb[kFallbackUnitDrain], dead};
     for (int i = 0; i < n; i++) out[i] = i < TREW_DEBUG_COUNTERS ? v[i] : 0;
     return 0;
 }
diff --git a/trew_amd/csrc/trew_common.hpp b/trew_amd/csrc/trew_common.hpp
--- a/trew_amd/csrc/trew_common.hpp
+++ b/trew_amd/csrc/trew_common.hpp
@@ -37,6 +37,9 @@
 };
 
 constexpr int kChunkCounterWord = 16;
+constexpr int kStoredPrefixWord = 1;
+constexpr int kDeadEntriesWord = 2;
+constexpr int kBoundNeedWords = 97;
 
 enum {
     kDiagOverflow = 0,
diff --git a/trew_amd/csrc/trew_kernels.hip b/trew_amd/csrc/trew_kernels.hip
--- a/trew_amd/csrc/trew_kernels.hip
+++ b/trew_amd/csrc/trew_kernels.hip
@@ -148,25 +148,47 @@
 }
 size_t bounds_entry_bytes() { return kBoundItemWords * sizeof(u32); }
 
-hipError_t launch_bounds(hipStream_t st, u32 n_cu, u64 n_units, const DevParams &P, const DevBatch &B, const u32 *wl, const u32 *wl_count,
-                         u32 wl_cap, u32 *bnd, u32 bnd_cap) {
+bool fill_bound_needs(const DevParams &P, u32 *table) {
+    bool usable = true;
+    for (int c = 0; c < kBoundNeedWords; c++) {
+        u32 need_lo = (u32) c + 1u, need_hi = (u32) c + 1u;
+        for (int m = c; m >= 0; m--) {
+            const double dm = (double) m, dc = (double) c;
+            const double tl = P.low * dc, th = P.high * dc;
+            const bool prod_lo = dm > tl, prod_hi = dm > th;
+            const bool amb = fabs(dm - tl) <= 1e-9 || fabs(dm - th) <= 1e-9;
+            const double ub = c ? dm / dc : 0.0;
+            const bool div_lo = ub >= P.low, div_hi = ub >= P.high;
+            if (!amb && (prod_lo != div_lo || prod_hi != div_hi)) usable = false;
+            if (div_lo) { if (need_lo != (u32) m + 1u) usable = false; need_lo = (u32) m; }
+            if (div_hi) { if (need_hi != (u32) m + 1u) usable = false; need_hi = (u32) m; }
+        }
+        table[c] = need_lo | (need_hi << 16);
+    }
+    return usable;
+}
+
+hipError_t launch_bounds(hipStream_t st, u32 n_cu, u64 n_units, const DevParams &P, const DevBatch &B, const u32 *wl, u32 *wl_count, u32 wl_cap,
+                         u32 *bnd, u32 bnd_cap, u32 *live, const u32 *need) {
     if (n_units == 0 || bnd_cap == 0) return hipSuccess;
-    const u64 most = (std::min<u64>(n_units, bnd_cap) * 2 + 63) / 64;
-    const u32 grid = (u32) std::min<u64>((u64) n_cu * 16ull, most);
-    hipLaunchKernelGGL(bounds_kernel<3>, dim3(grid), dim3(64), 0, st, P, B, wl, wl_count, wl_cap, bnd, bnd_cap);
+    const u64 per_block = 64ull * kBoundsWaves;
+    const u64 most = (std::min<u64>(n_units, bnd_cap) * 2 + per_block - 1) / per_block;
+    const u32 grid = (u32) std::min<u64>((u64) n_cu * 4ull, most);
+    hipLaunchKernelGGL(bounds_kernel<3>, dim3(grid), dim3((u32) per_block), 0, st, P, B, wl, wl_count, wl_cap, bnd, bnd_cap, live, need);
     return hipGetLastError();
 }
 
 hipError_t launch_exact(hipStream_t st, u32 n_cu, u64 n_units, const DevParams &P, const DevBatch &B, const DevTableG1 &T,
                         const u32 *wl, u32 *wl_count, u32 *wl_count_next, u32 wl_cap, const SegResults &R, u32 cap, u32 rawwords,
-                        u32 max_seg_len, bool share, const u32 *bnd, u32 bnd_cap) {
+                        u32 max_seg_len, bool share, const u32 *bnd, u32 bnd_cap, const u32 *live) {
     const bool wide = P.max_mer > 32;
     const u32 lds = exact_lds_bytes(cap, rawwords, wide ? 16u : 8u);
     const u32 bound_len = P.mode == TREW_MODE_LONG ? (u32) P.slice_len : max_seg_len;
     const int nw = (P.flags & TREW_FLAG_NO_FILTER) ? 0 : pick_nw(bound_len);
-    typedef void (*kern_t)(DevParams, DevBatch, DevTableG1, const u32 *, u32 *, u32 *, u32, SegResults, u32, u32, const u32 *, u32);
+    typedef void (*kern_t)(DevParams, DevBatch, DevTableG1, const u32 *, u32 *, u32 *, u32, SegResults, u32, u32, const u32 *, u32, const u32 *);
     kern_t fn = nullptr;
     if (!bounds_pass_applies(P, max_seg_len)) bnd = nullptr;
+    if (!bnd || !live) live = wl;
 #define TREW_PICK_MODE(NWV, WTV)                                                      \
     switch (P.mode) {                                                                 \
     case TREW_MODE_SHORT: fn = exact_kernel<NWV, TREW_MODE_SHORT, WTV>; break;        \
@@ -207,7 +229,7 @@
     if (const char *e = getenv("TREW_EXACT_WAVES_PER_CU")) per_cu = std::max(1, atoi(e));
     const u64 full = (u64) n_cu * (u64) per_cu;
     const u32 grid = (u32) std::min<u64>(full, std::max<u64>(n_units / 16, 64));
-    hipLaunchKernelGGL(fn, dim3(grid), dim3(64), lds, st, P, B, T, wl, wl_count, wl_count_next, wl_cap, R, cap, rawwords, bnd, bnd ? bnd_cap : 0u);
+    hipLaunchKernelGGL(fn, dim3(grid), dim3(64), lds, st, P, B, T, wl, wl_count, wl_count_next, wl_cap, R, cap, rawwords, bnd, bnd ? bnd_cap : 0u, live);
     return hipGetLastError();
 }
 
diff --git a/trew_amd/csrc/trew_launch.hpp b/trew_amd/csrc/trew_launch.hpp
--- a/trew_amd/csrc/trew_launch.hpp
+++ b/trew_amd/csrc/trew_launch.hpp
@@ -12,11 +12,12 @@
 void fill_thresholds(const DevParams &P, u32 uniform_length, int2 *table);
 hipError_t launch_exact(hipStream_t st, u32 n_cu, u64 n_units, const DevParams &P, const DevBatch &B, const DevTableG1 &T,
                         const u32 *wl, u32 *wl_count, u32 *wl_count_next, u32 wl_cap, const SegResults &R, u32 cap, u32 rawwords,
-                        u32 max_seg_len, bool share, const u32 *bnd, u32 bnd_cap);
+                        u32 max_seg_len, bool share, const u32 *bnd, u32 bnd_cap, const u32 *live);
 bool bounds_pass_applies(const DevParams &P, u32 max_seg_len);
 size_t bounds_entry_bytes();
-hipError_t launch_bounds(hipStream_t st, u32 n_cu, u64 n_units, const DevParams &P, const DevBatch &B, const u32 *wl, const u32 *wl_count,
-                         u32 wl_cap, u32 *bnd, u32 bnd_cap);
+hipError_t launch_bounds(hipStream_t st, u32 n_cu, u64 n_units, const DevParams &P, const DevBatch &B, const u32 *wl, u32 *wl_count, u32 wl_cap,
+                         u32 *bnd, u32 bnd_cap, u32 *live, const u32 *need);
+bool fill_bound_needs(const DevParams &P, u32 *table);
 u32 exact_lds_bytes_host(u32 cap, u32 rawwords, u32 wordbytes);
 hipError_t launch_g1_apply(hipStream_t st, const DevTable &T, const DevG1 &G, const DevBatch &B, int min_mer, const trew_hip_row *carry_in,
                            trew_hip_row *carry_out, u32 carry_cap);
```

New measurement: 2170, median of 6. +2.6%, better.
